# valauri/Littoral-Naval-Warfare-MARL

Hardware: AMD Instinct MI355X
Metric: env-steps/sec (whole node), 65536 parallel 4v4 envs on 100x100 grid (higher is better)
Workload: dtype f64+i32; 1 GPU; 65536 parallel 4v4 envs over 1 GPU(s) (65536 on rank 0), 100x100 Baltic grid, reference spawns, 40-step episodes with auto-reset, U[0,1)^4 f32 actions; global_envs=65536, envs_per_gpu=65536, agents=4v4, grid=100, spawns=reference, kernel_variant=default, los_mode=0, move_mode=0, parallelism=env-shard x1

## Files before the change

littoral-naval-warfare-marl_amd/csrc/lnw_device.h:

```cpp
#pragma once
#include <hip/hip_runtime.h>
#include <stdint.h>

namespace lnw {

constexpr int WAVE = 64;
constexpr int R_MV = 4;
constexpr int MV_W = 2 * R_MV + 1;
constexpr int MV_WORDS = 3;
constexpr int R_LOS = 40;
constexpr int LOS_W = 2 * R_LOS + 1;
constexpr int LOS_ROW_WORDS = 6;
constexpr int LOS_CELL_WORDS = LOS_W * LOS_ROW_WORDS;
constexpr int OPEN_CAP = 16;

enum { K_PYINT = 0, K_PYFLOAT = 1, K_F32 = 2, K_F64 = 3 };
enum { T_SMALL = 0, T_LARGE = 1, T_LS = 2, T_MEDIUM = 3 };

constexpr double PY_PI = 3.141592653589793;
constexpr double RAD2DEG = 180.0 / PY_PI;
constexpr double DEG2RAD = PY_PI / 180.0;

struct KParams {
  int discrete, landing_ops, aggressive, side_blue, trained_red;
  int move_thr, ew_thr, lz_x, lz_y;
  int episode_steps, auto_reset, los_mode, move_mode;
  int E, nb, nr, A, G, T, W16;
  int rng_mode;
  int act_dtype;
  int rew_f64;
  long long env_base;
  unsigned long long seed;
  double red_aggression;
  double hit64[2][9];
  float hit32[2][9];
  double d5[2][2];
  double den[2];
  double det_q[2];
  int box_lo[2], box_hi[2];
  int group_march;
  int xcd_remap;
  int wc[2];
  int epw;
  int store_wt;
  int atan_odd;
  int no_obs;
  long long obs_stride[2];
  int dbg_skip;
  int qdirect;
};

struct KState {
  uint32_t *pos;
  int32_t *radar;
  uint8_t *miss;
  uint8_t *mkind;
  uint8_t *alive;
  uint8_t *type;
  int32_t *steps;
  double *dist_lz;
  uint16_t *tl_cnt;
  uint16_t *tl;
  double *duct;
  int32_t *envi;
  unsigned long long *rng;
  uint32_t *err;
  double *bear_val;
  uint8_t *bear_ship;
  const double *atan_deg;
  const uint8_t *grid;
  const float *gridf;
  const float *winf;
  float *dummy;
  unsigned long long *prof;
  lnw_analytics ana;
  unsigned long long *ctr;
  const uint32_t *mask2;
  const uint32_t *mvtab;
  const uint32_t *lostab;
  const double *tape;
  const long long *tape_off;
  const int32_t *sp_types;
  const int32_t *sp_pos;
  const int32_t *sp_randls;
  const int32_t *sp_pos_env;
  int nmax;
};

__host__ __device__ inline uint32_t pack_pos(int x, int y) {
  return (uint32_t)(x & 0xffff) | ((uint32_t)(y & 0xffff) << 16);
}
__device__ inline int pos_x(uint32_t p) { return (int)(p & 0x7fff); }
__device__ inline int pos_y(uint32_t p) { return (int)((p >> 16) & 0x7fff); }

__device__ inline int kind_promote(int a, int b) {
  if (a == K_F64 || b == K_F64) return K_F64;
  if (a == K_F32 || b == K_F32) return K_F32;
  if (a == K_PYFLOAT || b == K_PYFLOAT) return K_PYFLOAT;
  return K_PYINT;
}

__device__ inline void philox10(uint32_t c[4], uint32_t k0, uint32_t k1) {
#pragma unroll
  for (int r = 0; r < 10; r++) {
    uint32_t hi0 = __umulhi(0xD2511F53u, c[0]), lo0 = 0xD2511F53u * c[0];
    uint32_t hi1 = __umulhi(0xCD9E8D57u, c[2]), lo1 = 0xCD9E8D57u * c[2];
    uint32_t n0 = hi1 ^ c[1] ^ k0, n2 = hi0 ^ c[3] ^ k1;
    c[0] = n0; c[1] = lo1; c[2] = n2; c[3] = lo0;
    k0 += 0x9E3779B9u;
    k1 += 0xBB67AE85u;
  }
}

__device__ inline void philox_u4(unsigned long long seed, unsigned long long ctr, float (&u)[4]) {
  uint32_t o[4] = {(uint32_t)ctr, (uint32_t)(ctr >> 32), 0x243F6A88u, 0x85A308D3u};
  philox10(o, (uint32_t)seed, (uint32_t)(seed >> 32));
#pragma unroll
  for (int k = 0; k < 4; k++) u[k] = (float)(o[k] >> 8) * 5.9604644775390625e-08f;
}

__device__ inline double u53(uint32_t a, uint32_t b) {
  return ((double)(a >> 5) * 67108864.0 + (double)(b >> 6)) / 9007199254740992.0;
}

__host__ __device__ inline unsigned long long tan_bits(double x) { return __builtin_bit_cast(unsigned long long, x); }
__host__ __device__ inline double tan_from_bits(unsigned long long b) { return __builtin_bit_cast(double, b); }
__host__ __device__ inline double tan_kernel_fd(double x, double y, int iy) {
  const double T0 = 3.33333333333334091986e-01, T1 = 1.33333333333201242699e-01,
               T2 = 5.39682539762260521377e-02, T3 = 2.18694882948595424599e-02,
               T4 = 8.86323982359930005737e-03, T5 = 3.59207910759131235356e-03,
               T6 = 1.45620945432529025516e-03, T7 = 5.88041240820264096874e-04,
               T8 = 2.46463134818469906812e-04, T9 = 7.81794442939557092300e-05,
               T10 = 7.14072491382608190305e-05, T11 = -1.85586374855275456654e-05,
               T12 = 2.59073051863633712884e-05;
  const double pio4 = 7.85398163397448278999e-01, pio4lo = 3.06161699786838301793e-17;
  const int hx = (int)(tan_bits(x) >> 32), ix = hx & 0x7fffffff;
  if (ix < 0x3e300000) {
    if (iy == 1) return x;
    return -1.0 / x;
  }
  const bool big = ix >= 0x3FE59428;
  if (big) {
    if (hx < 0) { x = -x; y = -y; }
    const double z = pio4 - x, w = pio4lo - y;
    x = z + w;
    y = 0.0;
  }
  double z = x * x, w = z * z;
  double r = T1 + w * (T3 + w * (T5 + w * (T7 + w * (T9 + w * T11))));
  double v = z * (T2 + w * (T4 + w * (T6 + w * (T8 + w * (T10 + w * T12)))));
  double s = z * x;
  r = y + z * (s * (r + v) + y);
  r += T0 * s;
  w = x + r;
  if (big) {
    v = (double)iy;
    return (double)(1 - ((hx >> 30) & 2)) * (v - 2.0 * (x - (w * w / (w + v) - r)));
  }
  if (iy == 1) return w;
  const double zz = tan_from_bits(tan_bits(w) & 0xffffffff00000000ull);
  v = r - (zz - x);
  const double a = -1.0 / w;
  const double t = tan_from_bits(tan_bits(a) & 0xffffffff00000000ull);
  s = 1.0 + t * zz;
  return t + a * (s + t * v);
}
__host__ __device__ inline double tan_fd(double x) {
  const int ix = (int)(tan_bits(x) >> 32) & 0x7fffffff;
// ... 395 lines not shown
```

littoral-naval-warfare-marl_amd/csrc/lnw_group.inc:

```

#ifdef LNW_GROUP_PROF
#define GPROF_MARK(t) unsigned long long t = __builtin_amdgcn_s_memrealtime()
#define GPROF_SET(t) (t) = __builtin_amdgcn_s_memrealtime()
#define GPROF_ADD(X, k, t)                                                   \
  do {                                                                       \
    const unsigned long long _n = __builtin_amdgcn_s_memrealtime();          \
    (X).gp[k] += _n - (t);                                                   \
    (t) = _n;                                                                \
  } while (0)
#define GPROF_FLUSH(X)                                                       \
  do {                                                                       \
    if ((X).S.prof && (threadIdx.x & (WAVE - 1)) == 0)                        \
      for (int _k = 0; _k < 8; _k++)                                         \
        atomicAdd(&(X).S.prof[(size_t)blockIdx.x * PROF_SLOTS + 16 + _k], (X).gp[_k]); \
  } while (0)
#else
#define GPROF_MARK(t) (void)0
#define GPROF_SET(t) (void)0
#define GPROF_ADD(X, k, t) (void)0
#define GPROF_FLUSH(X) (void)0
#endif

constexpr int GL = 16;
constexpr int GEPW = 32;
// ... 256 lines not shown
  g.pos = side ? gs[1].pos : gs[0].pos;
  g.shared = side ? gs[1].shared : gs[0].shared;
  const int jj = sub;
  const uint32_t posj = g.pos;
  const int gsh = (int)(threadIdx.x & (WAVE - 1)) & ~(GL - 1);
  GPROF_MARK(tq);
  const int ml = me - own0;
  const uint32_t vm = (movedm >> own0) & ((2u << ml) - 1u) & 0xffffu;
  auto sel = [&](uint32_t b) { return ((b & 0xffffu) & ~vm) | ((b >> 16) & vm); };
  const bool myradar = COLW(c.radar_cur, me) == 1;
  const bool nowalk = P.dbg_skip & 8192;
  const uint32_t dcol = nowalk ? 0u : (sel(g.c) | (myradar ? sel(g.r) : 0u));
  const uint32_t ecol = nowalk ? 0u : sel(g.w);
  GPROF_ADD(X, 4, tq);
  const int INF = 0x7fffffff;
  const int ij = dcol ? __builtin_ctz(dcol) : -1;
  int gj = ij >= 0 ? ij * nopp + jj : INF;
  if (g.shared) {
    int grow = -1, gcol = 0;
    for (uint32_t rows = group_or(dcol); rows; rows &= rows - 1) {
      const int i = __builtin_ctz(rows);
      const uint32_t m = group_ballot((dcol >> i) & 1u, gsh) & g.mates;
      if (grow < 0 && m) { grow = i; gcol = __builtin_ctz(m); }
    }
    gj = grow >= 0 ? grow * nopp + gcol : INF;
  }
  const bool rep = ij >= 0 && ij * nopp + jj == gj;
  const uint32_t low = (1u << jj) - 1u;
  const unsigned long long base = X.rng.ctr;
  auto slope_at = [&](int i, uint32_t pj, int r) {
    const uint32_t pi = COLW(c.pos_cur, own0 + i);
    const double a0 = bearing_tab(P, atab, half, pos_x(pj) - pos_x(pi), pos_y(pj) - pos_y(pi));
    const double gd = (P.dbg_skip & 262144) ? (double)(r & 7) * 0.25 - 1.0
                                            : X.rng.gauss_at(base + (unsigned long long)r);
    const double bearing = a0 + gd < 0 ? a0 + gd + 360.0 : a0 + gd;
    return (P.dbg_skip & 524288) ? bearing * 0.01 : tan_fd(bearing * DEG2RAD);
  };

  int nbear = 0, obs_n = 0, orank = 0, n = 0;
  uint32_t colb = 0;
  uint64_t it0 = 0, it1 = 0;
  int ni = 0;
  for (uint32_t rows = group_or(ecol | (rep ? 1u << ij : 0u)); rows; rows &= rows - 1) {
    const int i = __builtin_ctz(rows);
    const bool bb = ((ecol >> i) & 1u) && i * nopp + jj < gj;
    const uint32_t brow = group_ballot(bb, gsh);
    if (bb) {
      n++;
      colb |= 1u << i;
    }
    {
      const int cnt = __builtin_popcount(brow), t = (sub - nbear) & (GL - 1);
      if (t < cnt) {
        uint32_t mm = brow;
        int pos = 0, kk = t, cc = __builtin_popcount(mm & 0xffu);
        if (kk >= cc) { kk -= cc; mm >>= 8; pos += 8; }
        cc = __builtin_popcount(mm & 0xfu);
        if (kk >= cc) { kk -= cc; mm >>= 4; pos += 4; }
        cc = __builtin_popcount(mm & 0x3u);
        if (kk >= cc) { kk -= cc; mm >>= 2; pos += 2; }
        if (kk >= (int)(mm & 1u)) pos += 1;
        const uint64_t item = (uint64_t)(i | pos << 4 | ((nbear + t) & 0xff) << 8);
        if (ni < 4) it0 |= item << (16 * ni);
        else if (ni < 8) it1 |= item << (16 * (ni - 4));
        else ms[(i * nopp + pos) * GEPW] = slope_at(i, COLW(c.pos_cur, opp0 + pos), nbear + t);
        ni++;
      }
    }
    nbear += __builtin_popcount(brow);
    const bool rr = rep && ij == i;
    const uint32_t rrow = group_ballot(rr, gsh);
    if (rr) orank = obs_n + __builtin_popcount(rrow & low);
    obs_n += __builtin_popcount(rrow);
  }
  if (X.rng.mode == 1) {
    const long long avail = X.rng.tape_hi - X.rng.tape_lo - (long long)base;
    if (nbear > avail) X.rng.err |= 4u;
    X.rng.ctr += (unsigned long long)(nbear < avail ? nbear : (avail > 0 ? avail : 0));
  } else {
    X.rng.ctr += (unsigned long long)nbear;
  }
  GPROF_ADD(X, 5, tq);
  const uint32_t fixm = group_ballot(n >= 2, gsh);
  if (S.ctr && n >= 2) X.pooled += (unsigned)n;
  if (fixm && !(P.dbg_skip & 16384)) {
    auto item = [&](int q) { return (uint32_t)((q < 4 ? it0 >> (16 * q) : it1 >> (16 * (q - 4))) & 0xffffu); };
    for (int q = 0; q < ni; q += 2) {
      const uint32_t u1 = item(q), u2 = q + 1 < ni ? item(q + 1) : 0u;
      const bool f1 = (fixm >> ((u1 >> 4) & 15u)) & 1u, f2 = q + 1 < ni && ((fixm >> ((u2 >> 4) & 15u)) & 1u);
      if (!f1 && !f2) continue;
      const uint32_t v1 = f1 ? u1 : u2, v2 = f1 && f2 ? u2 : v1;
      const double m1 = slope_at((int)(v1 & 15u), COLW(c.pos_cur, opp0 + ((v1 >> 4) & 15u)), (int)(v1 >> 8));
      const double m2 = slope_at((int)(v2 & 15u), COLW(c.pos_cur, opp0 + ((v2 >> 4) & 15u)), (int)(v2 >> 8));
      ms[((v1 & 15u) * nopp + ((v1 >> 4) & 15u)) * GEPW] = m1;
      if (f1 && f2) ms[((v2 & 15u) * nopp + ((v2 >> 4) & 15u)) * GEPW] = m2;
    }
    wave_lds_sync();
  }
  const int fb = colb ? __builtin_ctz(colb) * nopp + jj : INF;
  int nt = 0, fxi = 0, fyi = 0;
  uint32_t err = 0;
  if (n >= 2 && !(P.dbg_skip & 16384)) {
    auto slope = [&](int i, double &x1, double &y1) {
      const uint32_t pi = COLW(c.pos_cur, own0 + i);
      x1 = pos_x(pi);
      y1 = pos_y(pi);
      return ms[(i * nopp + jj) * GEPW];
    };
    const int m = n - 1;
    FixAcc16 f;
    bool zero = false;
    double mprev = 0.0, xprev = 0.0, yprev = 0.0;
    uint32_t bits = colb;
    int k = 0;
    auto take = [&](double mt, double x1, double y1) {
      if (k > 0 && !zero) {
        if (mprev - mt == 0.0) {
          zero = true;
        } else {
          double x3, y3;
          fix_pair(mprev, mt, xprev, yprev, x1, y1, x3, y3);
          f.add(k - 1, m, x3, y3);
        }
      }
      k++;
      mprev = mt;
      xprev = x1;
      yprev = y1;
    };
    while (bits && !zero) {
      const int i1 = __builtin_ctz(bits);
      bits &= bits - 1;
      const bool two = bits != 0;
      const int i2 = two ? __builtin_ctz(bits) : i1;
      if (two) bits &= bits - 1;
      double x1, y1, x2, y2;
      const double m1 = slope(i1, x1, y1), m2 = slope(i2, x2, y2);
      take(m1, x1, y1);
      if (two) take(m2, x2, y2);
    }
    {
      double mx = 0.0, my = 0.0;
      if (zero) {
        err |= LNW_ERRF_ZERODIV;
      } else {
        f.mean(m, mx, my);
        if (!isfinite(mx) || !isfinite(my)) {
          err |= LNW_ERRF_NAN_ROUND;
        } else {
          const double rx = rint(mx), ry = rint(my);
          if (S.ana.ew_log) {
            const int ax = (int)fmin(fmax(rx, -32768.0), 32767.0), ay = (int)fmin(fmax(ry, -32768.0), 32767.0);
            ana_record(S.ana.ew_log, S.ana.ew_count, S.ana.ew_cap, (uint32_t)(P.env_base + env),
                       (uint32_t)X.step | (uint32_t)side << 16, COLW(c.pos_cur, me),
                       (uint32_t)(uint16_t)ax | (uint32_t)(uint16_t)ay << 16);
          }
          if (rx >= 0.0 && rx < (double)P.G && ry >= 0.0 && ry < (double)P.G) {
            fxi = (int)rx;
            fyi = (int)ry;
            for (int q = opp0; q < opp1; q++) {
              if (!COLB(c.alive0, q)) continue;
              const uint32_t pq = COLW(c.pos_cur, q);
              const int ddx = pos_x(pq) - fxi, ddy = pos_y(pq) - fyi;
              nt += ddx * ddx + ddy * ddy < 4 ? 1 : 0;
            }
          }
        }
      }
    }
  }
  GPROF_ADD(X, 6, tq);
  int off = obs_n, tot = obs_n;
#pragma unroll
  for (int q = 0; q < GL; q++) {
    const int fbg = __shfl(fb, gsh + q), ntg = __shfl(nt, gsh + q);
    tot += ntg;
    off += fbg < fb ? ntg : 0;
  }
  uint16_t *tl = S.tl + (size_t)me * P.T * E + env;
  const bool tls = !(P.dbg_skip & 1048576);
  if (rep && tls) tl[(size_t)orank * E] = (uint16_t)(pos_x(posj) | (pos_y(posj) << 8));
  if (nt > 0 && tls) {
    for (int q = opp0; q < opp1; q++) {
      if (!COLB(c.alive0, q)) continue;
      const uint32_t pq = COLW(c.pos_cur, q);
      const int ddx = pos_x(pq) - fxi, ddy = pos_y(pq) - fyi;
      if (ddx * ddx + ddy * ddy < 4) {
        tl[(size_t)off * E] = (uint16_t)(fxi | (fyi << 8));
        off++;
      }
    }
  }
  COLW(c.tcnt, me) = (uint32_t)tot;
  X.rng.err |= group_or(err);
  GPROF_ADD(X, 7, tq);
}

__device__ __forceinline__ float row_tail(const KParams &P, const Cols &c, const double *duct_col,
                                          int el, int k, int tk, uint32_t p, int own0, int ns,
                                          int kl, int t) {
  const double G = (double)P.G;
  if (t < 4) {
    if (t == 0) return (float)((double)pos_x(p) / G);
    if (t == 1) return (float)((double)pos_y(p) / G);
    if (t == 2) return (float)c.radar_cur[k * PAD + el];
    return (float)c.miss_cur[k * PADB + el] * (tk == T_SMALL ? 0.25f : 0.125f);
  }
  t -= 4;
  if (t < 4 * (ns - 1)) {
    const int s = t >> 2, comp = t & 3;
    const int il = s < kl ? s : s + 1, i = own0 + il;
    if (!c.alive0[i * PADB + el]) return 0.0f;
    const bool nw = il < kl;
    const uint32_t q = nw ? c.pos_cur[i * PAD + el] : c.pos_old[i * PAD + el];
    if (comp == 0) return (float)((double)pos_x(q) / G);
    if (comp == 1) return (float)((double)pos_y(q) / G);
    if (comp == 2) return (float)(nw ? c.radar_cur[i * PAD + el] : c.radar_old[i * PAD + el]);
    const int m = nw ? c.miss_cur[i * PADB + el] : c.miss_old[i * PADB + el];
    return (float)m * (c.type[i * PADB + el] == T_SMALL ? 0.25f : 0.125f);
  }
  t -= 4 * (ns - 1);
  if (t == 0) return (float)c.tcnt[k * PAD + el];
  if (t == 1) return tk == T_LS ? 1.0f : 0.0f;
  if (t == 2) return (float)(duct_col[el] / 2.0);
  return 0.0f;
}

__device__ __forceinline__ void group_rows(const KParams &P, const KState &S, const Cols &c,
                                           const double *duct_col, int el, long long env, int sub,
                                           float *obs_b, float *obs_r) {
  for (int sd = 0; sd < 2; sd++) {
    float *out = sd ? obs_r : obs_b;
    if (!out) continue;
    const int own0 = sd ? P.nb : 0, ns = sd ? P.nr : P.nb;
    const int D = side_D(P, sd), D4 = D / 4;
    f32x4 *base = (f32x4 *)(out + (size_t)env * ns * D);
// ... 109 lines not shown
  }
  if (tid < GEPW) {
    const double d = tid < nenv ? S.duct[env0 + tid] : 1.0;
    duct_col[tid] = d;
    r2col[tid] = max_range2(P, d);
  }
  __syncthreads();
  if (tid == 0) prof_stamp(S, 4);

  const int dt = P.act_dtype;
  bool pend = false;
  if (dt == LNW_ACT_F32)
    pend = group_move_phase<LNW_ACT_F32>(P, S, c, actions, row_kind, c.mask, env0, nenv, A, wid);
  else if (dt == LNW_ACT_F64)
    pend = group_move_phase<LNW_ACT_F64>(P, S, c, actions, row_kind, c.mask, env0, nenv, A, wid);
  else
    pend = group_move_phase<LNW_ACT_I32>(P, S, c, actions, row_kind, c.mask, env0, nenv, A, wid);
  if (__syncthreads_or(pend)) {
    if (wid == 0) move_astar_pass(P, S, c, nenv, A);
    __syncthreads();
  }

  if (tid == 0) prof_stamp(S, 1);
  if (valid) {
    Ctx X{P, S, c, slot, env, duct_col, make_rng(P, S, env), c.mask, E, r2col[slot], 0};
    X.leader = sub == 0;
    X.gsub = sub;
    X.gsh = (int)(threadIdx.x & (WAVE - 1)) & ~(GL - 1);
    GSide gs[2];
    uint32_t movedm;
    GPROF_MARK(tp);
    group_pair_tables(X, sub, gs, movedm);
    GPROF_ADD(X, 3, tp);
    Neut N{{0, 0}, {0u, 0u}};
    int ev[8];
#pragma unroll
    for (int q = 0; q < 8; q++) ev[q] = S.envi[q * E + env];
    X.step = ev[2];
    int hits[2] = {0, 0};
    int bsx = 0, bsy = 0, rsx = 0, rsy = 0;
    int nbp = 0, nrp = 0;
    GPROF_MARK(t0);
    for (int a = 0; a < A; a++) {
      const int lane = slot;
      const bool al = COLB(c.alive0, a) != 0;
      const int side = a >= nb;
      bool engage = false, moved = false;
      int destroyed = 0;
      if (al) {
        const uint32_t p0 = COLW(c.pos_cur, a);
        if (!side) {
          if (P.side_blue) { bsx += pos_x(p0); bsy += pos_y(p0); nbp++; }
        } else {
          rsx += pos_x(p0); rsy += pos_y(p0); nrp++;
        }
        const size_t row = ((size_t)env * A + a) * 4;
        const double a0 = COLW(c.act0, a);
        double a1 = COLW(c.act1, a);
        const int kind = COLB(c.akind, a);
        if (side && !P.trained_red) {
          if (X.rng.uniform() < P.red_aggression) {
            double v = X.rng.uniform();
            if (dt == LNW_ACT_F32) { float f = (float)v; ((float *)actions)[row + 1] = f; a1 = f; }
            else if (dt == LNW_ACT_F64) {
              if (kind == K_F32) v = (double)(float)v;
              ((double *)actions)[row + 1] = v; a1 = v;
            } else { ((int32_t *)actions)[row + 1] = 0; a1 = 0.0; }
          }
        }
        const double engagement = P.discrete ? rint(a1) : a1;
        const int keng = P.discrete ? K_PYINT : kind;
        const int mk = COLB(c.mkind, a);
        double thr_v;
        if (kind_promote(keng, mk) == K_F32)
          thr_v = (double)rintf((float)engagement * (float)COLB(c.miss_cur, a));
        else
          thr_v = rint(engagement * (double)COLB(c.miss_cur, a));
        if (!isfinite(thr_v)) { X.rng.err |= LNW_ERRF_NAN_ROUND; thr_v = 0.0; }
        engage = thr_v > 0.0;
        const int tn = (int)COLW(c.tcnt, a);
        if (engage && tn > 0 && !(P.dbg_skip & 65536)) {
          const uint16_t *tl = S.tl + (size_t)a * P.T * E + env;
          const int gsh = (int)(threadIdx.x & (WAVE - 1)) & ~(GL - 1);
          const bool par = !S.ana.heatmap && !S.ana.coldmap && !S.ana.launch && !S.ana.eng_log &&
                           !(P.dbg_skip & 32768);
          for (int q0 = 0; q0 < tn; q0 += GL) {
            const int q = q0 + sub;
            const int mine = q >= tn ? 0 : (tls && q < GTL) ? (int)tls[(a * GTL + q) * GEPW + slot]
                                                           : (int)tl[(size_t)q * E];
            const int nq = tn - q0 < GL ? tn - q0 : GL;
            if (par) {
              destroyed += fire_group_chunk(X, a, mine, nq, engagement, keng, N);
              continue;
            }
            for (int u = 0; u < nq; u++) {
              const uint16_t tg = (uint16_t)__shfl(mine, gsh + u);
              if (fire_dev<true>(X, a, tg & 0xff, tg >> 8, engagement, keng, N)) destroyed++;
            }
          }
        }
        if (side) ev[6] += destroyed; else ev[5] += destroyed;
        if (!isfinite(a0)) { X.rng.err |= LNW_ERRF_NAN_ROUND; COLW(c.radar_cur, a) = 0; }
        else {
          const double rr = rint(a0);
          COLW(c.radar_cur, a) = (int)fmin(fmax(rr, -2147483648.0), 2147483647.0);
        }
        const uint32_t pn = COLW(c.pos_new, a);
        moved = (pn & 0x80000000u) != 0;
        if (moved) COLW(c.pos_cur, a) = pn & 0x7fffffffu;
        GPROF_ADD(X, 0, t0);
        if (!(P.dbg_skip & 128)) get_obs_group(X, a, sub, gs, movedm, atab, half, ms);
        GPROF_SET(t0);
      }
      double r = 0.0;
      if (al && !(P.dbg_skip & 256))
        r = reward_core(P, S, c, slot, E, env, a, moved, engage, destroyed, dlz ? dlz + slot : nullptr, GEPW);
      GPROF_ADD(X, 1, t0);
      COLW(c.reward, a) = r;
      if (al) {
        if (!side) {
          if (P.side_blue ? destroyed > 0 : engage) COLB(c.eng, a) = 1;
        } else {
          if (!P.trained_red ? engage : destroyed > 1) COLB(c.eng, a) = 1;
        }
        if (side) hits[1] += destroyed; else hits[0] += destroyed;
      }
    }
    env_tail(P, S, c, slot, env, nb, A, N, ev, hits, nbp, nrp, bsx, bsy, rsx, rsy, X.rng, rew_b,
             rew_r, done_out, cog_out);
    if (S.ctr && X.pooled) atomicAdd(&S.ctr[3], (unsigned long long)X.pooled);
    GPROF_ADD(X, 2, t0);
    GPROF_FLUSH(X);
  }
  if (valid && !(P.dbg_skip & 1) && !P.no_obs) group_rows(P, S, c, duct_col, slot, env, sub, obs_b, obs_r);
}
```

littoral-naval-warfare-marl_amd/csrc/lnw_kernels.hip:

```cpp
#include <hip/hip_runtime.h>

#include <algorithm>
#include <cmath>
#include <cstdio>
#include <cstdlib>
#include <cstring>
#include <string>
#include <vector>

#include "lnw.h"
#include "lnw_device.h"

using namespace lnw;

typedef float f32x4 __attribute__((ext_vector_type(4)));
typedef int i32x4_t __attribute__((ext_vector_type(4)));

__device__ __forceinline__ void st_obs4(f32x4 *base, uint32_t i4, f32x4 v, bool wt) {
  if (wt) {
    const uint64_t bp = (uint64_t)(uintptr_t)base;
    const uint64_t ub = (uint64_t)(uint32_t)__builtin_amdgcn_readfirstlane((int)(uint32_t)bp) |
                        (uint64_t)(uint32_t)__builtin_amdgcn_readfirstlane((int)(uint32_t)(bp >> 32)) << 32;
    const __amdgpu_buffer_rsrc_t rs =
        __builtin_amdgcn_make_buffer_rsrc((void *)(uintptr_t)ub, 0, 0x7fffffff, 0x00020000);
// ... 141 lines not shown
  c.qstage1 = (float *)(base + L.qstage1);
  c.qlut = (float *)(base + L.qlut);
  c.qbig = (float *)(base + L.qbig);
  return c;
}

#define COLW(arr, a) ((arr)[(a) * PAD + lane])
#define COLB(arr, a) ((arr)[(a) * PADB + lane])

constexpr int PROF_SLOTS = 32;
__device__ inline unsigned long long prof_now(const KState &S) {
  return S.prof ? __builtin_amdgcn_s_memrealtime() : 0ull;
}
__device__ inline unsigned long long prof_acc(const KState &S, int slot, unsigned long long t0) {
  if (!S.prof) return 0ull;
  const unsigned long long t = __builtin_amdgcn_s_memrealtime();
  const unsigned long long m = __ballot(1);
  if ((int)(threadIdx.x & 63) == __ffsll((long long)m) - 1)
    atomicAdd(&S.prof[(size_t)blockIdx.x * PROF_SLOTS + slot], t - t0);
  return t;
}

struct Ctx {
  const KParams &P;
  const KState &S;
  Cols &c;
  int lane, env;
  const double *duct_col;
  Rng rng;
  const uint32_t *mask;
  long long E;
  int r2max;
  int step;
  uint64_t lpre[2];
  bool pre;
  uint32_t ptr_[2] = {0u, 0u}, ptc[2] = {0u, 0u}, ptw[2] = {0u, 0u};
  bool leader = true;
  int gsub = 0, gsh = 0;
  unsigned pooled = 0;
#ifdef LNW_GROUP_PROF
  unsigned long long gp[8] = {0, 0, 0, 0, 0, 0, 0, 0};
#endif
  __device__ double duct() const { return duct_col[lane]; }
};

__device__ inline void ana_record(uint32_t *log, uint32_t *count, long long cap, uint32_t w0,
                                  uint32_t w1, uint32_t w2, uint32_t w3) {
  const uint32_t i = atomicAdd(count, 1u);
  if ((long long)i < cap) {
    uint4 *r = (uint4 *)log + i;
    *r = make_uint4(w0, w1, w2, w3);
  }
}
__device__ inline void ana_map(uint32_t *map, uint32_t p) {
  const int x = pos_x(p), y = pos_y(p);
  if (map && x < 100 && y < 100) atomicAdd(&map[x * 100 + y], 1u);
}

__device__ inline int max_range2(const KParams &P, double duct) {
  int m = 16;
  for (int ti = 0; ti < 3; ti++)
    for (int tj = 0; tj < 3; tj++) {
      int r = radar_r(P, duct, ti, tj), e = ew_r(P, duct, ti, tj);
      m = max(m, max(r * r, e * e));
    }
  return m;
}

__device__ inline int floordiv7(int v) { int q = v / 7; if ((v % 7 != 0) && (v < 0)) q--; return q; }
__device__ inline int pymod7(int v) { int m = v % 7; if (m < 0) m += 7; return m; }

__device__ inline bool check_path_h(const KParams &P, const KState &S, int type, int sx, int sy,
                                    int tx, int ty, uint32_t *open, int ost) {
  if (tx < 0 || tx > 99 || ty < 0 || ty > 99) return false;
  int ox = tx - sx, oy = ty - sy;
  if (P.move_mode == 0 && ox >= -R_MV && ox <= R_MV && oy >= -R_MV && oy <= R_MV) {
    int cls = mv_cls(type);
    int bit = (ox + R_MV) * MV_W + (oy + R_MV);
    uint32_t w = S.mvtab[((size_t)cls * P.G * P.G + (size_t)sx * P.G + sy) * MV_WORDS + (bit >> 5)];
    return (w >> (bit & 31)) & 1u;
  }
  MaskBlocked mb{S.mask2, P.W16};
  bool sb = mb(sx, sy);
  if (S.ctr) atomicAdd(&S.ctr[2], 1ull);
  return check_path_dev(mb, sb, P.G, type, sx, sy, tx, ty, open, ost);
}

__device__ inline bool can_move_to_h(const KParams &P, const KState &S, int x, int y) {
  if (0 <= x && x < 100 && 0 <= y && y < 100) return !(cell_bits(S.mask2, P.W16, x, y) & 1u);
  return false;
}

__device__ inline uint32_t los_march_c(const KState &S, const uint32_t *mask, int W16, int x1,
                                       int y1, int x2, int y2) {
  if (!S.ctr) return los_march<true>(mask, W16, x1, y1, x2, y2);
  int n = 0;
  const uint32_t r = los_march<true>(mask, W16, x1, y1, x2, y2, &n);
  atomicAdd(&S.ctr[0], 1ull);
  atomicAdd(&S.ctr[1], (unsigned long long)n);
  return r;
}

__device__ inline uint32_t los_q(const KParams &P, const KState &S, const uint32_t *mask, int x1,
                                 int y1, int x2, int y2) {
  int dx = x2 - x1, dy = y2 - y1;
  if (P.los_mode != 1 && dx >= -R_LOS && dx <= R_LOS && dy >= -R_LOS && dy <= R_LOS) {
    int col = (dy + R_LOS) * 2;
    uint32_t w = S.lostab[((size_t)x1 * P.G + y1) * LOS_CELL_WORDS + (dx + R_LOS) * LOS_ROW_WORDS +
                          (col >> 5)];
    return (w >> (col & 31)) & 3u;
  }
  return los_march_c(S, mask, P.W16, x1, y1, x2, y2);
}

struct ObsAcc {
  int obs_n, norder;
};

__device__ inline void pair_after_los(Ctx &X, int i, int jj, int xi, int yi, int xj, int yj,
                                      bool rad_ok, bool close, bool ew_cand, uint32_t los,
                                      ObsAcc &acc);

__device__ inline void pair_detect(Ctx &X, int myradar, int i, int jj, int xi, int yi, int ti,
                                   int xj, int yj, int tj, int radj, int d2, ObsAcc &acc) {
  const KParams &P = X.P;
  const KState &S = X.S;
  Cols &c = X.c;
  const int lane = X.lane;
  int rr = radar_r(P, X.duct(), ti, tj), re = ew_r(P, X.duct(), ti, tj);
  bool rad_ok = myradar == 1 && d2 < rr * rr;
  bool close = d2 < 16;
  bool ew_cand = d2 < re * re && radj == 1;
  if (!(rad_ok || close || ew_cand)) return;
  pair_after_los(X, i, jj, xi, yi, xj, yj, rad_ok, close, ew_cand,
                 los_q(P, S, X.mask, xi, yi, xj, yj), acc);
}

__device__ inline bool pair_observe(Ctx &X, int xj, int yj, bool rad_ok, bool close, bool ew_cand,
                                    uint32_t los, ObsAcc &acc) {
  Cols &c = X.c;
  const int lane = X.lane;
  if (!(los & 1u)) return false;
  uint32_t pk = pack_pos(xj, yj);
  bool seen = false;
  for (int q = 0; q < acc.obs_n; q++) seen |= COLW(c.observed, q) == pk;
  if ((rad_ok || close) && !seen) {
    COLW(c.observed, acc.obs_n) = pk;
    acc.obs_n++;
    seen = true;
  }
  return ew_cand && (los & 2u) && !seen;
}

__device__ inline double bearing_deg(const KParams &P, const KState &S, int dx, int dy) {
  const bool tab = !(P.dbg_skip & 4096) && S.atan_deg && dx >= -R_LOS && dx <= R_LOS &&
                   dy >= -R_LOS && dy <= R_LOS;
  return tab ? S.atan_deg[(dy + R_LOS) * LOS_W + (dx + R_LOS)] : atan2((double)dy, (double)dx) * RAD2DEG;
}

struct BearPre {
  double v;
  bool tab;
};
__device__ inline BearPre bearing_pre(const KParams &P, const KState &S, int dx, int dy) {
  const bool tab = !(P.dbg_skip & 4096) && S.atan_deg && dx >= -R_LOS && dx <= R_LOS &&
                   dy >= -R_LOS && dy <= R_LOS;
  const double *p = tab ? S.atan_deg + (dy + R_LOS) * LOS_W + (dx + R_LOS) : (const double *)S.dummy;
  return {*p, tab};
}
__device__ inline double bearing_use(const BearPre &b, int dx, int dy) {
  return b.tab ? b.v : atan2((double)dy, (double)dx) * RAD2DEG;
}

__device__ inline double ew_bearing(const KParams &P, const KState &S, int xi, int yi, int xj, int yj,
                                    double distortion) {
  double bearing = bearing_deg(P, S, xj - xi, yj - yi);
  if (bearing + distortion < 0)
    bearing = bearing + distortion + 360.0;
  else
    bearing = bearing + distortion;
  return bearing;
}

__device__ inline void pair_after_los(Ctx &X, int i, int jj, int xi, int yi, int xj, int yj,
                                      bool rad_ok, bool close, bool ew_cand, uint32_t los,
                                      ObsAcc &acc) {
  const KState &S = X.S;
  Cols &c = X.c;
  const int lane = X.lane;
  if (pair_observe(X, xj, yj, rad_ok, close, ew_cand, los, acc)) {
    const double bearing = ew_bearing(X.P, S, xi, yi, xj, yj, X.rng.gauss());
    int k = COLB(c.bcnt, jj);
    if (k == 0) { COLB(c.border, acc.norder) = (uint8_t)jj; acc.norder++; }
    size_t slot = (size_t)(jj * S.nmax + k) * X.E + X.env;
    S.bear_val[slot] = bearing;
    S.bear_ship[slot] = (uint8_t)i;
    COLB(c.bcnt, jj) = (uint8_t)(k + 1);
  }
}

__device__ inline void pair_after_los_m(Ctx &X, int i, int jj, int opp0, int nopp, int xi, int yi,
                                        int xj, int yj, bool rad_ok, bool close, bool ew_cand,
                                        uint32_t los, ObsAcc &acc, uint64_t &obsm) {
  const KState &S = X.S;
  Cols &c = X.c;
  const int lane = X.lane;
  if (!(los & 1u)) return;
  bool seen = (obsm >> jj) & 1u;
  if ((rad_ok || close) && !seen) {
    const uint32_t pk = pack_pos(xj, yj);
    COLW(c.observed, acc.obs_n) = pk;
    acc.obs_n++;
    for (int k = 0; k < nopp; k++)
      if (COLW(c.pos_cur, opp0 + k) == pk) obsm |= 1ull << k;
    seen = true;
  }
  if (ew_cand && (los & 2u) && !seen) {
    const double bearing = ew_bearing(X.P, S, xi, yi, xj, yj, X.rng.gauss());
    int k = COLB(c.bcnt, jj);
    if (k == 0) { COLB(c.border, acc.norder) = (uint8_t)jj; acc.norder++; }
    size_t slot = (size_t)(jj * S.nmax + k) * X.E + X.env;
    S.bear_val[slot] = bearing;
    S.bear_ship[slot] = (uint8_t)i;
    COLB(c.bcnt, jj) = (uint8_t)(k + 1);
  }
}

struct FixAcc {
  double sumx = 0, sumy = 0, resx = 0, resy = 0;
  double r0x = 0, r1x = 0, r2x = 0, r3x = 0, r4x = 0, r5x = 0, r6x = 0, r7x = 0;
  double r0y = 0, r1y = 0, r2y = 0, r3y = 0, r4y = 0, r5y = 0, r6y = 0, r7y = 0;
  bool tail_started = false;
  __device__ void put(int r, bool acc, double x3, double y3) {
#define LNW_PUT(i)                                              \
  r##i##x = r == i ? (acc ? r##i##x + x3 : x3) : r##i##x;      \
  r##i##y = r == i ? (acc ? r##i##y + y3 : y3) : r##i##y;
    LNW_PUT(0) LNW_PUT(1) LNW_PUT(2) LNW_PUT(3) LNW_PUT(4) LNW_PUT(5) LNW_PUT(6) LNW_PUT(7)
#undef LNW_PUT
  }
  __device__ void add(int k, int m, double x3, double y3) {
    const int mblk = m - (m % 8);
    if (m < 8) {
      sumx += x3;
      sumy += y3;
    } else if (k < mblk) {
      put(k & 7, k >= 8, x3, y3);
    } else {
      if (!tail_started) { tree(); tail_started = true; }
      resx += x3;
      resy += y3;
    }
  }
  __device__ void tree() {
    resx = ((r0x + r1x) + (r2x + r3x)) + ((r4x + r5x) + (r6x + r7x));
    resy = ((r0y + r1y) + (r2y + r3y)) + ((r4y + r5y) + (r6y + r7y));
  }
  __device__ void mean(int m, double &mx, double &my) {
    if (m < 8) { mx = sumx / (double)m; my = sumy / (double)m; return; }
    if (!tail_started) tree();
    mx = resx / (double)m;
    my = resy / (double)m;
  }
};

__device__ inline void fix_pair(double m1, double m2, double x1, double y1, double x2, double y2,
                                double &x3, double &y3) {
  x3 = (m1 * x1 - m2 * x2 + y2 - y1) / (m1 - m2);
  y3 = m1 * (x3 - x1) + y1;
}

__device__ inline bool fix_mean_loop(Ctx &X, int jj, int n, double &mx, double &my) {
  const KState &S = X.S;
  Cols &c = X.c;
  const int lane = X.lane;
  auto slot = [&](int k) { return (size_t)(jj * S.nmax + k) * X.E + X.env; };
  const int m = n - 1;
  FixAcc f;
  for (int k = 0; k < m; k++) {
    uint8_t s1 = S.bear_ship[slot(k)], s2 = S.bear_ship[slot(k + 1)];
    double b1 = S.bear_val[slot(k)], b2 = S.bear_val[slot(k + 1)];
    uint32_t p1 = COLW(c.pos_cur, s1), p2 = COLW(c.pos_cur, s2);
    double m1 = tan_fd(b1 * DEG2RAD);
    double m2 = tan_fd(b2 * DEG2RAD);
    if (m1 - m2 == 0.0) return false;
    double x3, y3;
    fix_pair(m1, m2, pos_x(p1), pos_y(p1), pos_x(p2), pos_y(p2), x3, y3);
    f.add(k, m, x3, y3);
  }
  f.mean(m, mx, my);
  return true;
}

template <int BMAX>
__device__ inline bool fix_mean_batched(Ctx &X, int jj, int n, double &mx, double &my) {
  const KState &S = X.S;
  Cols &c = X.c;
  const int lane = X.lane;
  auto slot = [&](int k) { return (size_t)(jj * S.nmax + k) * X.E + X.env; };
  double bv[BMAX];
  int bs[BMAX];
#pragma unroll
  for (int k = 0; k < BMAX; k++) {
    bv[k] = 0.0;
    bs[k] = 0;
    if (k < n) { bv[k] = S.bear_val[slot(k)]; bs[k] = S.bear_ship[slot(k)]; }
  }
  double tv[BMAX], px[BMAX], py[BMAX];
#pragma unroll
  for (int k = 0; k < BMAX; k++) {
    tv[k] = 0.0;
    px[k] = py[k] = 0.0;
    if (k < n) {
      tv[k] = tan_fd(bv[k] * DEG2RAD);
      const uint32_t p = COLW(c.pos_cur, bs[k]);
      px[k] = pos_x(p);
      py[k] = pos_y(p);
    }
  }
  const int m = n - 1;
  FixAcc f;
  bool zero = false;
#pragma unroll
  for (int k = 0; k < BMAX - 1; k++) {
    if (k < m && !zero) {
      if (tv[k] - tv[k + 1] == 0.0) {
        zero = true;
      } else {
        double x3, y3;
        fix_pair(tv[k], tv[k + 1], px[k], py[k], px[k + 1], py[k + 1], x3, y3);
        f.add(k, m, x3, y3);
      }
    }
  }
  if (zero) return false;
  f.mean(m, mx, my);
  return true;
}

template <int BMAX, bool EXACT>
__device__ inline void finish_obs(Ctx &X, int me, int opp0, int opp1, const ObsAcc &acc) {
  const KParams &P = X.P;
  const KState &S = X.S;
  Cols &c = X.c;
  const int lane = X.lane;
  const long long E = X.E;
  const int env = X.env;
  const int obs_n = acc.obs_n, norder = acc.norder;
  const int T = P.T;
  uint16_t *tl = S.tl + (size_t)me * T * E + env;
  int tn = 0;
  for (int q = 0; q < obs_n; q++) {
    uint32_t pk = COLW(c.observed, q);
    tl[(size_t)tn * E] = (uint16_t)(pos_x(pk) | (pos_y(pk) << 8));
    tn++;
  }
  for (int o = 0; o < norder; o++) {
    int jj = COLB(c.border, o);
    int n = COLB(c.bcnt, jj);
    if (n < 2) continue;
    double mx, my;
    bool ok;
    if constexpr (EXACT) ok = fix_mean_batched<BMAX>(X, jj, n, mx, my);
    else ok = n <= BMAX ? fix_mean_batched<BMAX>(X, jj, n, mx, my) : fix_mean_loop(X, jj, n, mx, my);
    if (!ok) { X.rng.err |= LNW_ERRF_ZERODIV; continue; }
    if (!isfinite(mx) || !isfinite(my)) { X.rng.err |= LNW_ERRF_NAN_ROUND; continue; }
    double rx = rint(mx), ry = rint(my);
    if (S.ana.ew_log) {
      const int fx = (int)fmin(fmax(rx, -32768.0), 32767.0), fy = (int)fmin(fmax(ry, -32768.0), 32767.0);
      ana_record(S.ana.ew_log, S.ana.ew_count, S.ana.ew_cap, (uint32_t)(P.env_base + env),
                 (uint32_t)X.step | (uint32_t)(me >= P.nb) << 16, COLW(c.pos_cur, me),
                 (uint32_t)(uint16_t)fx | (uint32_t)(uint16_t)fy << 16);
    }
    if (!(rx >= 0.0 && rx < (double)P.G && ry >= 0.0 && ry < (double)P.G)) continue;
    int fxi = (int)rx, fyi = (int)ry;
    for (int j = opp0; j < opp1; j++) {
      if (!COLB(c.alive0, j)) continue;
      uint32_t pj = COLW(c.pos_cur, j);
      int ddx = pos_x(pj) - fxi, ddy = pos_y(pj) - fyi;
      if (ddx * ddx + ddy * ddy < 4) {
        tl[(size_t)tn * E] = (uint16_t)(fxi | (fyi << 8));
        tn++;
      }
    }
  }
  COLW(c.tcnt, me) = (uint32_t)tn;
}


template <int N, class T>
__device__ __forceinline__ T rsel(const T (&a)[N], int k) {
  T v = a[0];
#pragma unroll
  for (int q = 1; q < N; q++) v = k == q ? a[q] : v;
  return v;
}

__device__ __forceinline__ void march_pairs_ref(Ctx &X, int me) {
  const KParams &P = X.P;
  const Cols &c = X.c;
  const int lane = X.lane;
  const int side = me >= P.nb;
  const int own0 = side ? P.nb : 0, own1 = side ? P.A : P.nb;
  const int opp0 = side ? 0 : P.nb, opp1 = side ? P.nb : P.A;
  uint32_t acc = 0;
  for (int i = own0; i < own1; i++) {
    if (!COLB(c.alive0, i)) continue;
    const uint32_t pi = COLW(c.pos_cur, i);
    for (int j = opp0; j < opp1; j++) {
      if (!COLB(c.alive0, j)) continue;
      const uint32_t pj = COLW(c.pos_cur, j);
      int n = 0;
      acc += los_march<false>(X.mask, P.W16, pos_x(pi), pos_y(pi), pos_x(pj), pos_y(pj), &n);
      if (X.S.ctr) {
        atomicAdd(&X.S.ctr[0], 1ull);
        atomicAdd(&X.S.ctr[1], (unsigned long long)n);
      }
    }
  }
  if (acc == 0xffffffffu) X.S.dummy[lane] = 0.0f;
}

__device__ __forceinline__ void get_obs_dev(Ctx &X, int me) {
  const KParams &P = X.P;
  const KState &S = X.S;
  Cols &c = X.c;
  const int lane = X.lane;
  const int nb = P.nb, A = P.A;
  const int side = me >= nb;
  const int own0 = side ? nb : 0, own1 = side ? A : nb;
  const int opp0 = side ? 0 : nb, opp1 = side ? nb : A;
  const int nopp = opp1 - opp0, npair = (own1 - own0) * nopp;
  const int myradar = COLW(c.radar_cur, me);
  ObsAcc acc{0, 0};
  uint64_t obsm = 0;
  for (int q = 0; q < nopp; q++) COLB(c.bcnt, q) = 0;
  const double duct = X.duct();
  int rr_t[2][3], re_t[2][3];
#pragma unroll
  for (int mi = 0; mi < 2; mi++)
#pragma unroll
    for (int tj = 0; tj < 3; tj++) {
      const int ti = mi ? T_LARGE : T_SMALL;
      rr_t[mi][tj] = radar_r(P, duct, ti, tj);
      re_t[mi][tj] = ew_r(P, duct, ti, tj);
    }
  const unsigned long long tw = prof_now(S);
#pragma unroll 1
  for (int b0 = 0; b0 < npair; b0 += 16) {
    uint32_t radm = 0, closem = 0, ewm = 0, tabm = 0, marchm = 0;
    uint32_t wi[16];
    int ic = own0 + b0 / nopp, jc = opp0 + b0 % nopp;
    bool al_i = COLB(c.alive0, ic);
    uint32_t pi_c = COLW(c.pos_cur, ic);
    int mi_c = mast_cls(COLB(c.type, ic));
#pragma unroll
    for (int u = 0; u < 16; u++) {
      wi[u] = 0;
      const int b = b0 + u;
      const int j = jc;
      const bool ali = al_i;
      const uint32_t pi = pi_c;
      const int mi = mi_c;
      if (++jc == opp1) {
        jc = opp0;
        if (++ic < own1) {
          al_i = COLB(c.alive0, ic);
          pi_c = COLW(c.pos_cur, ic);
          mi_c = mast_cls(COLB(c.type, ic));
        }
      }
      if (b >= npair) continue;
      if (!ali || !COLB(c.alive0, j)) continue;
      const uint32_t pj = COLW(c.pos_cur, j);
      const int dx = pos_x(pj) - pos_x(pi), dy = pos_y(pj) - pos_y(pi);
      const int d2 = dx * dx + dy * dy;
      if (d2 >= X.r2max) continue;
      const int tj = rng_cls(COLB(c.type, j));
      const int rr0 = tj == 0 ? rr_t[0][0] : (tj == 1 ? rr_t[0][1] : rr_t[0][2]);
      const int rr1 = tj == 0 ? rr_t[1][0] : (tj == 1 ? rr_t[1][1] : rr_t[1][2]);
      const int re0 = tj == 0 ? re_t[0][0] : (tj == 1 ? re_t[0][1] : re_t[0][2]);
      const int re1 = tj == 0 ? re_t[1][0] : (tj == 1 ? re_t[1][1] : re_t[1][2]);
      const int rr = mi ? rr1 : rr0, re = mi ? re1 : re0;
      const bool rad_ok = myradar == 1 && d2 < rr * rr, close = d2 < 16;
      const bool ew_cand = d2 < re * re && COLW(c.radar_cur, j) == 1;
      if (!(rad_ok || close || ew_cand)) continue;
      radm |= (rad_ok ? 1u : 0u) << u;
      closem |= (close ? 1u : 0u) << u;
      ewm |= (ew_cand ? 1u : 0u) << u;
      if (P.los_mode != 1 && dx >= -R_LOS && dx <= R_LOS && dy >= -R_LOS && dy <= R_LOS) {
        tabm |= 1u << u;
        wi[u] = ((uint32_t)(pos_x(pi) * P.G + pos_y(pi)) * LOS_CELL_WORDS + (dx + R_LOS) * LOS_ROW_WORDS) *
                    32u + (dy + R_LOS) * 2;
      } else {
        marchm |= 1u << u;
      }
    }
    uint32_t losb = 0;
#pragma unroll
// ... 16 lines not shown
    }
  }
  const unsigned long long tf = prof_acc(S, 20, tw);
  finish_obs<16, false>(X, me, opp0, opp1, acc);
  prof_acc(S, 22, tf);
}


template <int NOWN, int NOPP, bool CW>
__device__ inline void finish_obs_t(Ctx &X, int me, int own0, int opp0, int obs_n,
                                    uint32_t firstbit, uint32_t bearm,
                                    const uint32_t (&pp)[NOPP], uint32_t oal = 0) {
  static_assert(NOWN < 9, "np.mean pairwise summation starts at 8 terms");
  const KParams &P = X.P;
  const KState &S = X.S;
  Cols &c = X.c;
  const int lane = X.lane;
  const long long E = X.E;
  const int env = X.env;
  const unsigned long long base = X.rng.ctr;
  const int nbear = __builtin_popcount(bearm);
  if (X.rng.mode == 1) {
    const long long avail = X.rng.tape_hi - X.rng.tape_lo - (long long)base;
    if (nbear > avail) X.rng.err |= 4u;
    X.rng.ctr += (unsigned long long)(nbear < avail ? nbear : (avail > 0 ? avail : 0));
  } else {
    X.rng.ctr += (unsigned long long)nbear;
  }
  uint16_t *tl = S.tl + (size_t)me * P.T * E + env;
  unsigned long long tq = prof_now(S);
  int tn = 0;
  if constexpr (CW) {
    for (uint32_t fb = firstbit; fb; fb &= fb - 1) {
      const uint32_t pk = COLW(c.pos_cur, opp0 + __builtin_ctz(fb) % NOPP);
      tl[(size_t)tn * E] = (uint16_t)(pos_x(pk) | (pos_y(pk) << 8));
      tn++;
    }
  } else {
    for (int q = 0; q < obs_n; q++) {
      uint32_t pk = COLW(c.observed, q);
      tl[(size_t)tn * E] = (uint16_t)(pos_x(pk) | (pos_y(pk) << 8));
      tn++;
    }
  }
  tq = prof_acc(S, 21, tq);
  if (!CW && bearm == 0) { COLW(c.tcnt, me) = (uint32_t)tn; return; }
  uint32_t colj = 0;
#pragma unroll
  for (int i = 0; i < NOWN; i++) colj |= 1u << (i * NOPP);
  uint32_t need = 0;
#pragma unroll
  for (int j = 0; j < NOPP; j++) {
    const uint32_t bj = bearm & (colj << j);
    if (__builtin_popcount(bj) < 2) continue;
#pragma unroll
    for (int i = 0; i < NOWN; i++) need |= ((bj >> (i * NOPP + j)) & 1u) << (j * NOWN + i);
  }
  if (S.prof) {
    const int cnt = __builtin_popcount(need);
    int s = 0, mx = 0;
    for (int b = 4; b >= 0; b--) {
      s += __popcll(__ballot((cnt >> b) & 1)) << b;
      if (__ballot(cnt >= (mx | (1 << b)))) mx |= 1 << b;
    }
    const unsigned long long m = __ballot(1);
    if ((int)(threadIdx.x & 63) == __ffsll((long long)m) - 1) {
      atomicAdd(&S.prof[(size_t)blockIdx.x * PROF_SLOTS + 24], (unsigned long long)s);
      atomicAdd(&S.prof[(size_t)blockIdx.x * PROF_SLOTS + 25], (unsigned long long)mx);
      atomicAdd(&S.prof[(size_t)blockIdx.x * PROF_SLOTS + 26], (unsigned long long)__popcll(m));
    }
  }
  static_assert(NOPP <= 4, "fix cells packed 16 bits per opponent");
  uint64_t fixw = 0;
  uint32_t fok = 0;
  int curj = -1, cnt = 0;
  bool zero = false;
  double sumx = 0.0, sumy = 0.0, mprev = 0.0, xprev = 0.0, yprev = 0.0;
  auto flush = [&]() {
    if (curj < 0) return;
    if (zero) { X.rng.err |= LNW_ERRF_ZERODIV; return; }
    const double mx = sumx / (double)(cnt - 1), my = sumy / (double)(cnt - 1);
    if (!isfinite(mx) || !isfinite(my)) { X.rng.err |= LNW_ERRF_NAN_ROUND; return; }
    const double rx = rint(mx), ry = rint(my);
    if (S.ana.ew_log) {
      const int fx = (int)fmin(fmax(rx, -32768.0), 32767.0), fy = (int)fmin(fmax(ry, -32768.0), 32767.0);
      ana_record(S.ana.ew_log, S.ana.ew_count, S.ana.ew_cap, (uint32_t)(P.env_base + env),
                 (uint32_t)X.step | (uint32_t)(me >= P.nb) << 16, COLW(c.pos_cur, me),
                 (uint32_t)(uint16_t)fx | (uint32_t)(uint16_t)fy << 16);
    }
    if (!(rx >= 0.0 && rx < (double)P.G && ry >= 0.0 && ry < (double)P.G)) return;
    fixw |= (uint64_t)((uint32_t)(int)rx | (uint32_t)(int)ry << 8) << (16 * curj);
    fok |= 1u << curj;
  };
  if constexpr (CW) {
  auto setup = [&](int t, int &dx, int &dy, int &j, double &x1, double &y1, int &k) {
    j = t / NOWN;
    const int i = t - j * NOWN, b = i * NOPP + j;
    const uint32_t pi = COLW(c.pos_cur, own0 + i), pj = COLW(c.pos_cur, opp0 + j);
    dx = pos_x(pj) - pos_x(pi);
    dy = pos_y(pj) - pos_y(pi);
    x1 = pos_x(pi);
    y1 = pos_y(pi);
    k = __builtin_popcount(bearm & ((1u << b) - 1u));
  };
  auto accum = [&](int j, double m, double x1, double y1) {
    if (j != curj) {
      flush();
      curj = j; cnt = 0; zero = false; sumx = sumy = 0.0;
    }
    if (cnt > 0 && !zero) {
      if (mprev - m == 0.0) {
        zero = true;
      } else {
        double x3, y3;
        fix_pair(mprev, m, xprev, yprev, x1, y1, x3, y3);
        sumx += x3;
        sumy += y3;
      }
    }
    cnt++;
    mprev = m; xprev = x1; yprev = y1;
  };
  const unsigned long long act = __ballot(1);
  const int ncnt = __builtin_popcount(need);
  int wmax = 0;
#pragma unroll
  for (int b = 4; b >= 0; b--)
    if (__ballot(ncnt >= (wmax | (1 << b)))) wmax |= 1 << b;
  if (NOWN * NOPP > 2 && wmax > 2 && !(P.dbg_skip & 131072)) {
    const int nact = __popcll(act);
    const int rank = (int)__builtin_amdgcn_mbcnt_hi((uint32_t)(act >> 32),
                                                    __builtin_amdgcn_mbcnt_lo((uint32_t)act, 0u));
    int excl = 0, total = 0;
#pragma unroll
    for (int b = 0; b < 5; b++) {
      const unsigned long long bb = __ballot((ncnt >> b) & 1);
      excl += (int)__builtin_amdgcn_mbcnt_hi((uint32_t)(bb >> 32),
                                             __builtin_amdgcn_mbcnt_lo((uint32_t)bb, 0u)) << b;
      total += __popcll(bb) << b;
    }
    if (S.ctr && rank == 0) atomicAdd(&S.ctr[3], (unsigned long long)total);
    uint8_t *lor = (uint8_t *)c.observed;
    uint16_t *exr = (uint16_t *)(lor + WAVE);
    uint32_t *fixt = (uint32_t *)(lor + 3 * WAVE);
    lor[rank] = (uint8_t)lane;
    exr[rank] = (uint16_t)excl;
    asm volatile("s_waitcnt lgkmcnt(0)" ::: "memory");
    const int prevl = rank > 0 ? (int)lor[rank - 1] : lane;
    const int lastl = 63 - __builtin_clzll(act);
    const bool tape = X.rng.mode == 1;
    constexpr uint32_t SEGM = (1u << NOWN) - 1u;
    auto locate = [&](int g, int &s, int &i, int &j, uint32_t &nsj, unsigned long long &drw,
                      uint32_t &pi, uint32_t &pj) {
      int lo = 0;
#pragma unroll
      for (int st = 32; st; st >>= 1)
        if (lo + st < nact && (int)exr[lo + st] <= g) lo += st;
      s = lor[lo];
      const int kk = g - (int)exr[lo];
      uint32_t ns = (uint32_t)__shfl((int)need, s);
      const uint32_t bs = (uint32_t)__shfl((int)bearm, s);
      drw = __shfl(base, s);
      uint32_t w = ns;
      for (int q = 0; q < kk; q++) w &= w - 1;
      const int t = __builtin_ctz(w);
      j = t / NOWN;
      i = t - j * NOWN;
      const int b = i * NOPP + j;
      drw += (unsigned long long)__builtin_popcount(bs & ((1u << b) - 1u));
      nsj = (ns >> (j * NOWN)) & SEGM;
      pi = c.pos_cur[(own0 + i) * PAD + s];
      pj = c.pos_cur[(opp0 + j) * PAD + s];
    };
    auto draw = [&](int s, unsigned long long d) -> double {
      const int es = env - lane + s;
      if (tape) {
        if (!S.tape_off) return 0.0;
        const long long p = S.tape_off[es] + (long long)d;
        return p < S.tape_off[es + 1] ? S.tape[p] : 0.0;
      }
      const unsigned long long gid = (unsigned long long)(P.env_base + es);
      return X.rng.gauss_philox(d, (uint32_t)gid, (uint32_t)(gid >> 32));
    };
    auto finish = [&](int s, int j, int n, double sx, double sy, bool z, int stp) {
      uint32_t w = 0;
      if (z) {
        w = 1u << 17;
      } else {
        const double mx = sx / (double)(n - 1), my = sy / (double)(n - 1);
        if (!isfinite(mx) || !isfinite(my)) {
          w = 1u << 18;
        } else {
          const double rx = rint(mx), ry = rint(my);
          if (S.ana.ew_log) {
            const int fx = (int)fmin(fmax(rx, -32768.0), 32767.0), fy = (int)fmin(fmax(ry, -32768.0), 32767.0);
            ana_record(S.ana.ew_log, S.ana.ew_count, S.ana.ew_cap, (uint32_t)(P.env_base + env - lane + s),
                       (uint32_t)stp | (uint32_t)(me >= P.nb) << 16, c.pos_cur[me * PAD + s],
                       (uint32_t)(uint16_t)fx | (uint32_t)(uint16_t)fy << 16);
          }
          if (rx >= 0.0 && rx < (double)P.G && ry >= 0.0 && ry < (double)P.G)
            w = (uint32_t)(int)rx | (uint32_t)(int)ry << 8 | 1u << 16;
        }
      }
      fixt[j * WAVE + s] = w;
    };
    double cm = 0.0, csx = 0.0, csy = 0.0;
    uint32_t cp = 0;
    int cz = 0;
    for (int r0 = 0; r0 < total; r0 += 2 * nact) {
      const int gA = r0 + 2 * rank, gB = gA + 1;
      int sA, iA, jA, sB, iB, jB;
      uint32_t nA, nB, piA, pjA, piB, pjB;
      unsigned long long dA, dB;
      locate(min(gA, total - 1), sA, iA, jA, nA, dA, piA, pjA);
      locate(min(gB, total - 1), sB, iB, jB, nB, dB, piB, pjB);
      const int dx1 = pos_x(pjA) - pos_x(piA), dy1 = pos_y(pjA) - pos_y(piA);
      const int dx2 = pos_x(pjB) - pos_x(piB), dy2 = pos_y(pjB) - pos_y(piB);
      const BearPre b1 = bearing_pre(P, S, dx1, dy1), b2 = bearing_pre(P, S, dx2, dy2);
      double a1 = b1.v, a2 = b2.v;
      if (!(b1.tab && b2.tab)) {
        a1 = bearing_use(b1, dx1, dy1);
        a2 = bearing_use(b2, dx2, dy2);
      }
      const double gg1 = draw(sA, dA), gg2 = draw(sB, dB);
      const double br1 = a1 + gg1 < 0 ? a1 + gg1 + 360.0 : a1 + gg1;
      const double br2 = a2 + gg2 < 0 ? a2 + gg2 + 360.0 : a2 + gg2;
      const double mA = tan_fd(br1 * DEG2RAD), mB = tan_fd(br2 * DEG2RAD);
      const bool fA = !(nA & ((1u << iA) - 1u)), fB = !(nB & ((1u << iB) - 1u));
      const bool lA = !(nA >> (iA + 1)), lB = !(nB >> (iB + 1));
      const double tm = __shfl(mB, prevl);
      const uint32_t tp = (uint32_t)__shfl((int)piB, prevl);
      const double pm = rank > 0 ? tm : cm;
      const uint32_t pp = rank > 0 ? tp : cp;
      double xA = 0.0, yA = 0.0, xB = 0.0, yB = 0.0;
      const bool zA = !fA && pm - mA == 0.0, zB = !fB && mA - mB == 0.0;
      if (!fA && !zA)
        fix_pair(pm, mA, pos_x(pp), pos_y(pp), pos_x(piA), pos_y(piA), xA, yA);
      if (!fB && !zB)
        fix_pair(mA, mB, pos_x(piA), pos_y(piA), pos_x(piB), pos_y(piB), xB, yB);
      double sxA = 0.0, syA = 0.0, sxB = 0.0, syB = 0.0;
      bool ZA = false, ZB = false;
#pragma unroll
      for (int pass = 0; pass < (NOWN - 1) / 2 + 1; pass++) {
        const double qx = __shfl(sxB, prevl), qy = __shfl(syB, prevl);
        const int qz = __shfl((int)ZB, prevl);
        const double inx = rank > 0 ? qx : csx, iny = rank > 0 ? qy : csy;
        const bool inz = (rank > 0 ? qz : cz) != 0;
        sxA = fA ? 0.0 : inx + xA;
        syA = fA ? 0.0 : iny + yA;
        ZA = !fA && (inz || zA);
        sxB = fB ? 0.0 : sxA + xB;
        syB = fB ? 0.0 : syA + yB;
        ZB = !fB && (ZA || zB);
      }
      int stA = 0, stB = 0;
      if (S.ana.ew_log) {
        stA = __shfl(X.step, sA);
        stB = __shfl(X.step, sB);
      }
      if (gA < total && lA) finish(sA, jA, __builtin_popcount(nA), sxA, syA, ZA, stA);
      if (gB < total && lB) finish(sB, jB, __builtin_popcount(nB), sxB, syB, ZB, stB);
      cm = __shfl(mB, lastl);
      cp = (uint32_t)__shfl((int)piB, lastl);
      csx = __shfl(sxB, lastl);
      csy = __shfl(syB, lastl);
      cz = __shfl((int)ZB, lastl);
    }
    asm volatile("s_waitcnt lgkmcnt(0)" ::: "memory");
#pragma unroll
    for (int j = 0; j < NOPP; j++) {
      if (__builtin_popcount((need >> (j * NOWN)) & SEGM) < 2) continue;
      const uint32_t w = fixt[j * WAVE + lane];
      if (w & (1u << 17)) X.rng.err |= LNW_ERRF_ZERODIV;
      else if (w & (1u << 18)) X.rng.err |= LNW_ERRF_NAN_ROUND;
      else if (w & (1u << 16)) {
        fixw |= (uint64_t)(w & 0xffffu) << (16 * j);
        fok |= 1u << j;
      }
    }
  } else
  while (need) {
    const int t1 = __builtin_ctz(need);
    need &= need - 1;
    const bool two = need != 0;
    const int t2 = two ? __builtin_ctz(need) : t1;
    if (two) need &= need - 1;
    int dx1, dy1, j1, k1, dx2, dy2, j2, k2;
    double x1, y1, x2, y2;
    setup(t1, dx1, dy1, j1, x1, y1, k1);
    setup(t2, dx2, dy2, j2, x2, y2, k2);
    const BearPre b1 = bearing_pre(P, S, dx1, dy1), b2 = bearing_pre(P, S, dx2, dy2);
    double a1 = b1.v, a2 = b2.v;
    if (!(b1.tab && b2.tab)) {
      a1 = bearing_use(b1, dx1, dy1);
      a2 = bearing_use(b2, dx2, dy2);
    }
    const double g1 = X.rng.gauss_at(base + (unsigned long long)k1);
    const double g2 = X.rng.gauss_at(base + (unsigned long long)k2);
    const double br1 = a1 + g1 < 0 ? a1 + g1 + 360.0 : a1 + g1;
    const double br2 = a2 + g2 < 0 ? a2 + g2 + 360.0 : a2 + g2;
    const double m1 = tan_fd(br1 * DEG2RAD), m2 = tan_fd(br2 * DEG2RAD);
    accum(j1, m1, x1, y1);
    if (two) accum(j2, m2, x2, y2);
  }
  } else {
  while (need) {
    const int t = __builtin_ctz(need);
    need &= need - 1;
    const int j = t / NOWN, i = t - j * NOWN, b = i * NOPP + j;
    const uint32_t pi = COLW(c.pos_cur, own0 + i), pj = COLW(c.pos_cur, opp0 + j);
    const int dx = pos_x(pj) - pos_x(pi), dy = pos_y(pj) - pos_y(pi);
    const double a0 = bearing_deg(P, S, dx, dy);
    if (j != curj) {
      flush();
      curj = j; cnt = 0; zero = false; sumx = sumy = 0.0;
    }
    const int k = __builtin_popcount(bearm & ((1u << b) - 1u));
    const double g = X.rng.gauss_at(base + (unsigned long long)k);
    const double bearing = a0 + g < 0 ? a0 + g + 360.0 : a0 + g;
    const double m = tan_fd(bearing * DEG2RAD);
    const double x1 = pos_x(pi), y1 = pos_y(pi);
    if (cnt > 0 && !zero) {
      if (mprev - m == 0.0) {
        zero = true;
      } else {
        double x3, y3;
        fix_pair(mprev, m, xprev, yprev, x1, y1, x3, y3);
        sumx += x3;
        sumy += y3;
      }
    }
    cnt++;
    mprev = m; xprev = x1; yprev = y1;
  }
  }
  flush();
  tq = prof_acc(S, 22, tq);
  uint32_t rem = bearm, done = 0;
  while (rem) {
// ... 366 lines not shown
template <bool GRP = false>
__device__ inline int check_target_dev(Ctx &X, int side, int tx, int ty) {
  const KParams &P = X.P;
  Cols &c = X.c;
  const int lane = X.lane;
  int opp0 = side ? 0 : P.nb, opp1 = side ? P.nb : P.A;
  if constexpr (GRP) {
    const int j = opp0 + X.gsub;
    bool hit = false;
    if (j < opp1 && COLB(c.alive0, j)) {
      const uint32_t pj = COLW(c.pos_cur, j);
      const int dx = pos_x(pj) - tx, dy = pos_y(pj) - ty;
      hit = dx * dx + dy * dy <= 12;
    }
    const uint32_t m = (uint32_t)(__ballot(hit) >> X.gsh) & 0xffffu;
    return m ? opp0 + __builtin_ctz(m) : -1;
  }
  for (int j = opp0; j < opp1; j++) {
    if (!COLB(c.alive0, j)) continue;
    uint32_t pj = COLW(c.pos_cur, j);
    int dx = pos_x(pj) - tx, dy = pos_y(pj) - ty;
    if (dx * dx + dy * dy <= 12) return j;
  }
  return -1;
}

struct Neut {
  int cnt[2];
  uint32_t mask[2];
};

template <bool GRP = false>
__device__ inline bool fire_dev(Ctx &X, int a, int tx, int ty, double salvo, int ksalvo, Neut &N) {
  const KParams &P = X.P;
  Cols &c = X.c;
  const int lane = X.lane;
  const int side = a >= P.nb;
  int t = check_target_dev<GRP>(X, side, tx, ty);
  if (t < 0) return false;
  uint32_t pt = COLW(c.pos_cur, t), pa = COLW(c.pos_cur, a);
  int dx = pos_x(pt) - pos_x(pa), dy = pos_y(pt) - pos_y(pa);
  bool hit = false, missile = false;
  int n = 0;
  if (dx * dx + dy * dy < 4) {
    hit = true;
  } else {
    int miss = COLB(c.miss_cur, a);
    if (miss == 0) return false;
    int mk = COLB(c.mkind, a);
    double u1, u2;
    X.rng.uniform2(u1, u2);
    bool detected = !(u1 < (COLW(c.radar_cur, t) == 1 ? P.det_q[0] : P.det_q[1]));
    int hp = detected ? 0 : 1;
    double num;
    int kn;
    if (!P.discrete) {
      int kp = kind_promote(mk, ksalvo);
      if (kp == K_F32) {
        num = (double)rintf((float)miss * (float)salvo);
        kn = K_F32;
      } else {
        num = rint((double)miss * salvo);
        kn = K_F64;
      }
    } else {
      num = COLB(c.type, a) == T_SMALL ? salvo : salvo * 2.0;
      kn = K_PYINT;
    }
    if (num > (double)miss) { num = (double)miss; kn = mk; }
    n = (int)num;
    COLB(c.miss_cur, a) = (uint8_t)(miss - n);
    COLB(c.mkind, a) = (uint8_t)kind_promote(mk, kn);
    if (n < 0 || n > 8) { X.rng.err |= LNW_ERRF_MISSILES; n = n < 0 ? 0 : 8; }
    if (kn == K_F32)
      hit = (float)u2 < hit_sel(P.hit32, hp, n);
    else
      hit = u2 < hit_sel(P.hit64, hp, n);
    missile = true;
  }
  if (hit && X.leader) {
    const KState &S = X.S;
    if (missile) {
      if (side == (P.side_blue ? 0 : 1)) {
        ana_map(S.ana.heatmap, pa);
        ana_map(S.ana.coldmap, pt);
      }
      if (S.ana.launch) ana_map(S.ana.launch + side * 10000, pa);
    }
    if (S.ana.eng_log)
      ana_record(S.ana.eng_log, S.ana.eng_count, S.ana.eng_cap, (uint32_t)(P.env_base + X.env),
                 (uint32_t)X.step | (uint32_t)side << 16 | (uint32_t)n << 24, pa, pt);
  }
  if (hit) {
    int ts = t >= P.nb;
    N.cnt[ts]++;
    N.mask[ts] |= 1u << (t - (ts ? P.nb : 0));
  }
  return hit;
}

__device__ inline int fire_draws(Ctx &X, int a, double salvo, int ksalvo) {
  const KParams &P = X.P;
  Cols &c = X.c;
  const int lane = X.lane;
  const int side = a >= P.nb;
  const int tn = (int)COLW(c.tcnt, a);
  int miss = COLB(c.miss_cur, a), mk = COLB(c.mkind, a), nd = 0;
  const uint16_t *tl = X.S.tl + (size_t)a * P.T * X.E + X.env;
  const uint32_t pa = COLW(c.pos_cur, a);
  for (int q = 0; q < tn; q++) {
    const uint16_t tg = tl[(size_t)q * X.E];
    const int t = check_target_dev<false>(X, side, tg & 0xff, tg >> 8);
    if (t < 0) continue;
    const uint32_t pt = COLW(c.pos_cur, t);
    const int dx = pos_x(pt) - pos_x(pa), dy = pos_y(pt) - pos_y(pa);
    if (dx * dx + dy * dy < 4 || miss == 0) continue;
    double num;
    int kn;
    if (!P.discrete) {
      if (kind_promote(mk, ksalvo) == K_F32) {
        num = (double)rintf((float)miss * (float)salvo);
        kn = K_F32;
      } else {
        num = rint((double)miss * salvo);
        kn = K_F64;
      }
    } else {
      num = COLB(c.type, a) == T_SMALL ? salvo : salvo * 2.0;
      kn = K_PYINT;
    }
    if (num > (double)miss) { num = (double)miss; kn = mk; }
    miss = (miss - (int)num) & 0xff;
    mk = kind_promote(mk, kn);
    nd += 2;
  }
  return nd;
}

__device__ __forceinline__ double reward_core(const KParams &P, const KState &S, Cols &c, int lane,
                                              long long E, int env, int a, bool moved, bool engage,
                                              int n_hit, const double *dlz = nullptr, int dlz_stride = 0) {
  size_t ai = (size_t)a * E + env;
  int steps = COLW(c.steps, a) + 1;
  COLW(c.steps, a) = steps;
  int tl_n = (int)COLW(c.tcnt, a);
  double r = 0.0;
  if (tl_n > 0) r += (double)(tl_n * 3);
  if (moved) r += 1.0;
  else r = fmax(r - 0.5, 0.0);
  if (tl_n > 0 && !engage) r = r / 2.0;
  else if (tl_n > 0 && engage && n_hit == 0) r += 0.5;
  r += (double)(n_hit * 10);
  int t = COLB(c.type, a);
  uint32_t p = COLW(c.pos_cur, a);
  int x = pos_x(p), y = pos_y(p);
  bool red = a >= P.nb;
  if (red && t != T_LS && !P.aggressive) {
    if (steps > 14) {
      if (x < 19 || x > 55 || y < 40 || y > 70) r = fmax(r - 2.0, 0.0);
      else r += 1.0;
    }
  }
  if (red && P.aggressive && t != T_LS) {
    int dx = x - 15, dy = y - 60;
    double nom = fmax(sqrt((double)(dx * dx + dy * dy)), 1.0);
    double d = (1.0 / (nom / (mast_cls(t) ? P.den[1] : P.den[0]))) * 1.0;
    r += d;
  }
  if (t == T_LS) {
    int dx = x - P.lz_x, dy = y - P.lz_y;
    double dl = sqrt((double)(dx * dx + dy * dy));
    if (dl > 0) {
      double cur = (P.dbg_skip & 2097152) ? 1e9 : (dlz ? dlz[a * dlz_stride] : S.dist_lz[ai]);
      if (dl < cur) { r += 1.0; S.dist_lz[ai] = dl; }
      else r -= 1.0;
    } else {
      r += 100.0;
    }
    if (dl == 0) r += 100.0;
    else r += log10(100.0 / dl) * 5.0;
  }
  return r;
}

__device__ inline double reward_dev(Ctx &X, int a, bool moved, bool engage, int n_hit) {
  return reward_core(X.P, X.S, X.c, X.lane, X.E, X.env, a, moved, engage, n_hit);
}

__device__ __forceinline__ void reset_env_dev(const KParams &P, const KState &S, int env, Rng &rng) {
  const long long E = P.E;
  double duct = 1.0 + rng.beta13();
  S.duct[env] = duct;
  bool box = P.box_hi[0] > P.box_lo[0] && P.box_hi[1] > P.box_lo[1];
  unsigned long long box_ctr = ((unsigned long long)(uint32_t)S.envi[7 * E + env]) << 32;
  for (int a = 0; a < P.A; a++) {
    size_t ai = (size_t)a * E + env;
    int t = S.sp_types[a];
    int x, y;
    if (S.sp_pos_env) {
      x = S.sp_pos_env[((size_t)env * P.A + a) * 2];
      y = S.sp_pos_env[((size_t)env * P.A + a) * 2 + 1];
    } else {
      x = S.sp_pos[2 * a];
      y = S.sp_pos[2 * a + 1];
    }
    if (box) {
      for (int tries = 0; tries < 64; tries++) {
        uint32_t o[4];
        o[0] = (uint32_t)box_ctr;
        o[1] = (uint32_t)(box_ctr >> 32);
        o[2] = rng.g0;
        o[3] = rng.g1 ^ 0x80000000u;
        philox10(o, rng.k0 ^ 0x5bd1e995u, rng.k1);
        box_ctr++;
        int bx = P.box_lo[0] + (int)(o[0] % (uint32_t)(P.box_hi[0] - P.box_lo[0]));
        int by = P.box_lo[1] + (int)(o[1] % (uint32_t)(P.box_hi[1] - P.box_lo[1]));
        if (!(cell_bits(S.mask2, P.W16, bx, by) & 1u)) { x = bx; y = by; break; }
      }
    }
    if (S.sp_randls[a]) {
      x = rng.randint(98, 99);
      y = rng.randint(48, 56);
    }
    S.pos[ai] = pack_pos(x, y);
    S.radar[ai] = 1;
    S.miss[ai] = (uint8_t)missiles0(t);
    S.mkind[ai] = K_PYINT;
    S.alive[ai] = 1;
    S.type[ai] = (uint8_t)t;
    S.steps[ai] = 0;
    S.tl_cnt[ai] = 0;
    double dl = 0.0;
    if (t == T_LS) {
      int dx = x - P.lz_x, dy = y - P.lz_y;
      dl = sqrt((double)(dx * dx + dy * dy));
    }
    S.dist_lz[ai] = dl;
  }
  S.envi[0 * E + env] = P.nb;
  S.envi[1 * E + env] = P.nr;
  S.envi[2 * E + env] = 0;
  S.envi[3 * E + env] = 0;
  S.envi[4 * E + env] = 0;
  S.envi[7 * E + env] = S.envi[7 * E + env] + 1;
}

__device__ inline Rng make_rng(const KParams &P, const KState &S, int env) {
  Rng r;
  r.mode = P.rng_mode;
  r.k0 = (uint32_t)P.seed;
  r.k1 = (uint32_t)(P.seed >> 32);
  unsigned long long gid = (unsigned long long)(P.env_base + env);
  r.g0 = (uint32_t)gid;
  r.g1 = (uint32_t)(gid >> 32);
  r.ctr = S.rng[env];
  r.err = 0;
  r.tape = S.tape;
  if (P.rng_mode == 1 && S.tape_off) {
    r.tape_lo = S.tape_off[env];
    r.tape_hi = S.tape_off[env + 1];
  } else {
    r.tape_lo = r.tape_hi = 0;
  }
  return r;
}

__device__ __forceinline__ void build_row(const KParams &P, const KState &S, const Cols &c, const double *duct_col,
                          int el, int k, float *row, const float *xg, bool only_observed) {
  const int side = k >= P.nb;
  const int own0 = side ? P.nb : 0;
  const int ns = side ? P.nr : P.nb;
  const int kl = k - own0;
  const int D = side_D(P, side);
  const int G = P.G;
  if (!c.alive0[k * PADB + el] || (only_observed && !c.obsd[k * PADB + el])) {
    for (int d = 0; d < D; d++) row[d] = 0.0f;
    return;
  }
  const int tk = c.type[k * PADB + el];
  const uint32_t p = c.pos_cur[k * PAD + el];
  const int px = pos_x(p), py = pos_y(p);
  int idx;
  if (tk == T_LS || tk == T_MEDIUM) {
    const f32x4 *w = (const f32x4 *)(S.winf + ((size_t)win_cls(tk) * G * G + (size_t)(px * G + py)) * 52);
    f32x4 v[7];
#pragma unroll
    for (int q = 0; q < 7; q++) v[q] = w[q];
    f32x4 *r4 = (f32x4 *)row;
#pragma unroll
    for (int q = 0; q < 6; q++) r4[q] = v[q];
    row[24] = v[6].x;
    idx = 25;
  } else {
    const f32x4 *w = (const f32x4 *)(S.winf + (size_t)(px * G + py) * 52);
    f32x4 v[13];
#pragma unroll
    for (int q = 0; q < 13; q++) v[q] = w[q];
    f32x4 *r4 = (f32x4 *)row;
#pragma unroll
    for (int q = 0; q < 12; q++) r4[q] = v[q];
    row[48] = v[12].x;
    idx = 49;
  }
  row[idx++] = xg[px];
  row[idx++] = xg[py];
  row[idx++] = (float)c.radar_cur[k * PAD + el];
  row[idx++] = (float)c.miss_cur[k * PADB + el] * (tk == T_SMALL ? 0.25f : 0.125f);
  for (int il = 0; il < ns; il++) {
    if (il == kl) continue;
    const int i = own0 + il;
    if (c.alive0[i * PADB + el]) {
      const bool nw = il < kl;
      const uint32_t q = nw ? c.pos_cur[i * PAD + el] : c.pos_old[i * PAD + el];
      row[idx] = xg[pos_x(q)];
      row[idx + 1] = xg[pos_y(q)];
      row[idx + 2] = (float)(nw ? c.radar_cur[i * PAD + el] : c.radar_old[i * PAD + el]);
      const int m = nw ? c.miss_cur[i * PADB + el] : c.miss_old[i * PADB + el];
      row[idx + 3] = (float)m * (c.type[i * PADB + el] == T_SMALL ? 0.25f : 0.125f);
    } else {
      row[idx] = row[idx + 1] = row[idx + 2] = row[idx + 3] = 0.0f;
    }
    idx += 4;
  }
  row[idx++] = (float)c.tcnt[k * PAD + el];
  row[idx++] = tk == T_LS ? 1.0f : 0.0f;
  row[idx++] = (float)(duct_col[el] / 2.0);
  for (; idx < D; idx++) row[idx] = 0.0f;
}

__device__ inline void copy_side(const float *stage, float *out, int ns, int D, int ne, long long genv0,
                                 long long stride = 0) {
  if (!out) return;
  const int lane = threadIdx.x & (WAVE - 1);
  const int S4 = stage_stride(ns) >> 2;
  const int D4 = D >> 2;
  const int n4 = ne * ns * D4;
  const f32x4 *st4 = (const f32x4 *)stage;
  if (stride && stride != (long long)ns * D) {
    const int per = ns * D4;
    for (int i = lane; i < n4; i += WAVE) {
      const int e = i / per, q = i - e * per, r = e * ns + q / D4;
      ((f32x4 *)(out + (genv0 + e) * stride))[q] = st4[r * S4 + (q - (q / D4) * D4)];
    }
    return;
  }
// ... 745 lines not shown
          for (int a = 0; a < A; a++) {
            if (a < nb) COLW(c.reward, a) = COLW(c.reward, a) - COLW(c.reward, a);
            else COLW(c.reward, a) += 100.0;
          }
          ev[3] += 1;
        }
      }
    }
  }
  ev[2] = ev[2] + 1;
  if (nbp > 0 && nrp > 0) {
    double bx = (double)bsx / nbp, by = (double)bsy / nbp, rx = (double)rsx / nrp, ry = (double)rsy / nrp;
    cog = sqrt((bx - rx) * (bx - rx) + (by - ry) * (by - ry));
  }
  *cog_p = cog;
  return done;
}

__device__ __forceinline__ bool env_resets(const KParams &P, int done, int steps_env) {
  return P.auto_reset && (done == 0 || (P.episode_steps > 0 && steps_env >= P.episode_steps));
}

__device__ __forceinline__ void env_tail(const KParams &P, const KState &S, Cols &c, int lane, int env,
                                         int nb, int A, const Neut &N, int (&ev)[8],
                                         const int (&hits)[2], int nbp, int nrp, int bsx, int bsy,
                                         int rsx, int rsy, Rng &rng, float *rew_b, float *rew_r,
                                         int32_t *done_out, float *cog_out, bool quiet = false) {
  const long long E = P.E;
  const int nr = A - nb;
  double cog;
  const int done = env_tail_core(P, c, lane, nb, A, N, ev, hits, nbp, nrp, bsx, bsy, rsx, rsy, &cog, quiet);
  const int steps_env = ev[2];
  if (P.rew_f64) {
    for (int a = 0; a < nb; a++)
      if (rew_b) ((double *)rew_b)[(size_t)env * nb + a] = COLW(c.reward, a);
    for (int a = 0; a < nr; a++)
      if (rew_r) ((double *)rew_r)[(size_t)env * nr + a] = COLW(c.reward, nb + a);
    if (cog_out) ((double *)cog_out)[env] = cog;
  } else {
    for (int a = 0; a < nb; a++)
      if (rew_b) rew_b[(size_t)env * nb + a] = (float)COLW(c.reward, a);
    for (int a = 0; a < nr; a++)
      if (rew_r) rew_r[(size_t)env * nr + a] = (float)COLW(c.reward, nb + a);
    if (cog_out) cog_out[env] = (float)cog;
  }
  if (done_out) done_out[env] = done;
  prof_stamp(S, 2);
  const bool do_reset = env_resets(P, done, steps_env);
  for (int a = 0; a < A; a++) {
    size_t ai = (size_t)a * E + env;
    int side = a >= nb;
    bool killed = (N.mask[side] >> (a - (side ? nb : 0))) & 1u;
    S.pos[ai] = COLW(c.pos_cur, a);
    S.radar[ai] = COLW(c.radar_cur, a);
    S.steps[ai] = COLW(c.steps, a);
    if (quiet) continue;
    S.miss[ai] = COLB(c.miss_cur, a);
    S.mkind[ai] = COLB(c.mkind, a);
    S.alive[ai] = COLB(c.alive0, a) && !killed;
    S.tl_cnt[ai] = (uint16_t)COLW(c.tcnt, a);
  }
  if (quiet) {
    S.envi[2 * E + env] = ev[2];
    if (done == 0) {
      S.envi[3 * E + env] = ev[3];
      S.envi[4 * E + env] = ev[4];
    }
  } else {
#pragma unroll
    for (int q = 0; q < 8; q++) S.envi[q * E + env] = ev[q];
  }
  if (do_reset) reset_env_dev(P, S, env, rng);
  if (!quiet || !P.trained_red || do_reset) S.rng[env] = rng.ctr;
  if (rng.err) S.err[env] |= rng.err;
}

#include "lnw_quiet.inc"

extern __shared__ __attribute__((aligned(16))) char lds_dyn[];

template <int NB, int NR, bool CW, bool REFW, int UN, bool PS, bool SL>
__device__ __forceinline__ void step_body(
    const KParams &P, KState S, void *actions, const uint8_t *row_kind, float *obs_b, float *obs_r,
    float *rew_b, float *rew_r, int32_t *done_out, float *cog_out) {
  static_assert(UN == 1 || (NB > 0 && EPW == WAVE && !REFW), "units need the two-wave templated kernel");
  const int unit = UN > 1 ? (int)(threadIdx.x / (2 * WAVE)) : 0;
  const int lane = threadIdx.x & (WAVE - 1);
  const int wid = UN > 1 ? (int)((threadIdx.x / WAVE) & 1) : (int)(threadIdx.x / WAVE);
  const int epw = P.epw;
  const int env0 = (UN > 1 ? blockIdx.x * UN + unit : xcd_chunk(P, (int)blockIdx.x, (int)gridDim.x)) * epw;
  if (UN > 1 && S.prof) S.prof += (size_t)(blockIdx.x * (UN - 1) + unit) * PROF_SLOTS;
  const int env = env0 + lane;
  const long long E = P.E;
  const bool valid = lane < epw && env < E;
  const int nenv = (E - env0) < epw ? (int)(E - env0) : epw;
  constexpr bool ST = NB > 0;
  const int nb = ST ? NB : P.nb, nr = ST ? NR : P.nr;
  const int A = nb + nr;
  const int qbig_rows = !(ST && NB == NR && EPW == WAVE && P.los_mode == 0) ? 0
                        : SL ? (P.qdirect ? WAVE : 0)
                             : (epw * NB <= WAVE ? epw * NB : 0);
  LdsLayout L = lds_layout(A, nb, nr, S.nmax, P.G * P.W16, P.G, qbig_rows);
  const int lstride = (L.total + 15) & ~15;
  Cols c = carve(lds_dyn + unit * lstride, L);
  __shared__ double duct_all[UN][WAVE];
  __shared__ int prog_all[UN], qclaim_all[UN];
  __shared__ int r2_all[UN][WAVE];
  __shared__ int ushare[2];
  double *duct_col = duct_all[unit];
  int &prog = prog_all[unit], &qclaim = qclaim_all[unit];
  int *r2col = r2_all[unit];
  if (UN > 1 && threadIdx.x == 0) { ushare[0] = 0; ushare[1] = 0; }
  const bool psplit = PS && CW && NB == 4 && NR == 4 && UN == 1 && EPW == WAVE && P.los_mode == 0 &&
                      !(P.dbg_skip & 515) && !(P.dbg_skip & 16384);
  const bool emit = ST && P.los_mode != 1 && nenv == WAVE && !(P.dbg_skip & 3) && !P.no_obs && !psplit;
  constexpr int NW = ST && EPW == WAVE ? 2 : 1;
  if (NW == 1 && wid == 1) return;
  constexpr int MAXPRE = 4;
  const int dt = P.act_dtype;
  const bool pre = ST && NW == 2 && dt == LNW_ACT_F32 && !(P.dbg_skip & 4) && !(P.dbg_skip & 8388608);
  f32x4 vpre[MAXPRE];
  if (pre) preload_rows_f32<NW, MAXPRE>(actions, env0, nenv, A, wid, vpre);
  int evp[8] = {0, 0, 0, 0, 0, 0, 0, 0};
  Rng rngp{};
  const bool evpre = ST && !CW && NW == 2 && UN == 1 && NB == NR && epw * NB <= WAVE && P.los_mode == 0 &&
                     !(P.dbg_skip & (1 << 29));
  if (evpre && wid == 0 && valid) {
#pragma unroll
    for (int q = 0; q < 8; q++) evp[q] = S.envi[q * E + env];
    rngp = make_rng(P, S, env);
  }
  if (wid == 0) {
    prof_stamp(S, 0);
    prof_put(S, 30, (unsigned long long)__builtin_amdgcn_s_getreg((3 << 11) | 20));
    prof_put(S, 31, (unsigned long long)__builtin_amdgcn_s_getreg((31 << 11) | 4));
  } else if (wid == 1) {
    prof_put(S, 29, (unsigned long long)__builtin_amdgcn_s_getreg((31 << 11) | 4));
  }

  stage_mask<NW>(P, S, c.mask, (int)threadIdx.x - unit * NW * WAVE);
  const uint32_t *mask = c.mask;
  load_state<NB + NR, NW>(P, S, c, lane, env, valid, wid);
  double duct = valid ? S.duct[env] : 1.0;
  if (wid == 0) {
    duct_col[lane] = duct;
    r2col[lane] = max_range2(P, duct);
    if (lane == 0) prog = -1;
  }
  __syncthreads();
  if (wid == 0) prof_stamp(S, 4);

  bool pend = false;
  if (!(P.dbg_skip & 4)) {
    if (pre)
      pend = move_phase_pre<NW, MAXPRE>(P, S, c, actions, row_kind, mask, env0, nenv, A, wid, vpre);
    else if (dt == LNW_ACT_F32)
      pend = move_phase<LNW_ACT_F32, NW>(P, S, c, actions, row_kind, mask, env0, nenv, A, wid);
    else if (dt == LNW_ACT_F64)
      pend = move_phase<LNW_ACT_F64, NW>(P, S, c, actions, row_kind, mask, env0, nenv, A, wid);
    else
      pend = move_phase<LNW_ACT_I32, NW>(P, S, c, actions, row_kind, mask, env0, nenv, A, wid);
  }
  const bool qcap = ST && P.los_mode == 0 && !(P.dbg_skip & 3) && !(P.dbg_skip & 512);
  const bool astar = NW > 1 ? __syncthreads_or(pend) != 0 : true;
  if constexpr (ST && NW > 1) {
    if (qcap) {
      if (wid == 0) prof_stamp(S, 6);
      if (astar) {
        if (wid == 0) move_astar_pass(P, S, c, nenv, A);
        __syncthreads();
      }
      if (wid == 0) prof_stamp(S, 7);
      bool wq;
      if (NB == NR && UN == 1 && P.epw * NB <= WAVE && !(P.dbg_skip & 268435456))
        wq = wg_quiet_spread_t<NB, NB>(P, c, lane, r2col);
      else
        wq = __all(env_quiet_t<NB, NR>(P, c, lane, r2col[lane]));
      if (wid == 0) prof_stamp(S, 8);
#ifdef LNW_DIAG
      if (P.dbg_skip & (1 << 24)) {
        wq = __all(env_quiet_t<NB, NR>(P, c, lane, r2col[lane] + (P.dbg_skip >> 30)));
        if (wid == 0) prof_stamp(S, 12);
      }
#endif
      if (__builtin_expect(wq, 1)) {
        if constexpr (UN > 1)
          quiet_step_units_t<NB, NR, UN>(P, S, c, lds_dyn, L, lstride, unit, lane, env, wid, duct_all,
                                         ushare, actions, obs_b, obs_r, rew_b, rew_r, done_out, cog_out,
                                         env0, valid);
        else
          quiet_step_t<NB, NR, SL>(P, S, c, lane, env, wid, duct_col, &qclaim, actions, obs_b, obs_r, rew_b,
                               rew_r, done_out, cog_out, env0, nenv, valid, evpre, evp, rngp);
        return;
      }
      if (UN > 1) __syncthreads();
    }
  }
#ifdef LNW_PROBE_QUIET_ONLY
  if constexpr (ST && NW > 1) return;
#endif
  const bool phase_o = !((P.dbg_skip & 1) || emit || P.no_obs);
  if (wid == 1 && !psplit) {
    if constexpr (ST) {
      if (emit) emit_wave_t<NB>(P, S, c, duct_col, &prog, obs_b, obs_r, env0);
    }
    prof_stamp(S, 5);
    return;
  }
  if (!qcap && astar && !(P.dbg_skip & 4)) {
    move_astar_pass(P, S, c, nenv, A);
    wave_lds_sync();
  }

  prof_stamp(S, 1);
  if (valid && !(P.dbg_skip & 2)) {
    if (emit) publish_progress(&prog, 0);
// ... 256 lines not shown
            thr_v = (double)rintf((float)engagement * (float)COLB(c.miss_cur, a));
          else
            thr_v = rint(engagement * (double)COLB(c.miss_cur, a));
          if (!isfinite(thr_v)) { X.rng.err |= LNW_ERRF_NAN_ROUND; thr_v = 0.0; }
          engage = thr_v > 0.0;
          int tn = (int)COLW(c.tcnt, a);
          if (engage && tn > 0 && !(P.dbg_skip & 65536)) {
            const uint16_t *tl = S.tl + (size_t)a * P.T * E + env;
            if constexpr (CW) {
              for (int q0 = 0; q0 < tn; q0 += 8) {
                uint64_t pk0 = 0, pk1 = 0;
#pragma unroll
                for (int u = 0; u < 8; u++) {
                  const uint64_t v = q0 + u < tn ? (uint64_t)tl[(size_t)(q0 + u) * E] : 0ull;
                  if (u < 4) pk0 |= v << (16 * u);
                  else pk1 |= v << (16 * (u - 4));
                }
                const int nq = tn - q0 < 8 ? tn - q0 : 8;
                for (int u = 0; u < nq; u++) {
                  const uint16_t tg = (uint16_t)((u < 4 ? pk0 : pk1) >> (16 * (u & 3)));
                  if (fire_dev(X, a, tg & 0xff, tg >> 8, engagement, keng, N)) destroyed++;
                }
              }
            } else {
              uint16_t nx = tl[0];
              for (int q = 0; q < tn; q++) {
                const uint16_t tg = nx;
                if (q + 1 < tn) nx = tl[(size_t)(q + 1) * E];
                if (fire_dev(X, a, tg & 0xff, tg >> 8, engagement, keng, N)) destroyed++;
              }
            }
          }
          if (side) ev[6] += destroyed; else ev[5] += destroyed;
          if (!isfinite(a0)) { X.rng.err |= LNW_ERRF_NAN_ROUND; COLW(c.radar_cur, a) = 0; }
          else {
            double rr = rint(a0);
            COLW(c.radar_cur, a) = (int)fmin(fmax(rr, -2147483648.0), 2147483647.0);
          }
          uint32_t pn = COLW(c.pos_new, a);
          moved = (pn & 0x80000000u) != 0;
          if (moved) COLW(c.pos_cur, a) = pn & 0x7fffffffu;
        }
        tp[0] += prof_now(S) - t0;
        t0 = prof_now(S);
        if (al && !(P.dbg_skip & 128)) {
          if constexpr (REFW) march_pairs_ref(X, a);
          if constexpr (ST) {
            if (!side) get_obs_t<NB, NR, CW>(X, a, 0, NB);
            else get_obs_t<NR, NB, CW>(X, a, NB, 0);
          } else {
            get_obs_dev(X, a);
          }
        }
        tp[2] += prof_now(S) - t0;
        t0 = prof_now(S);
        double r = 0.0;
        if (al && !(P.dbg_skip & 256)) r = reward_dev(X, a, moved, engage, destroyed);
        COLW(c.reward, a) = r;
        if (al) {
          if (!side) {
            if (P.side_blue ? destroyed > 0 : engage) COLB(c.eng, a) = 1;
          } else {
            if (!P.trained_red ? engage : destroyed > 1) COLB(c.eng, a) = 1;
          }
          hits[side] += destroyed;
        }
        tp[3] += prof_now(S) - t0;
        if (emit) publish_progress(&prog, a + 1);
        if (a < 8) prof_stamp(S, 6 + a);
      }
    }
    env_tail(P, S, c, lane, env, nb, A, N, ev, hits, nbp, nrp, bsx, bsy, rsx, rsy, X.rng, rew_b,
             rew_r, done_out, cog_out);
    if (S.prof && lane == 0)
      for (int q = 0; q < 4; q++) prof_put(S, 16 + q, tp[q]);
  }
  prof_stamp(S, 3);
  if (!phase_o) return;
  __syncthreads();
  if constexpr (ST) write_obs_t<NB, NR>(P, S, c, duct_col, obs_b, obs_r, env0, nenv);
  else write_obs(P, S, c, duct_col, obs_b, obs_r, env0, nenv, false);
}

template <int NB, int NR, bool CW = false, bool REFW = false, int UN = 1, bool PS = false, bool SL = false>
__global__ __launch_bounds__(NB > 0 && EPW == WAVE ? 2 * WAVE * UN : WAVE, NB > 0 ? 2 : 1) void step_kernel(
    KParams P, KState S, void *actions, const uint8_t *row_kind, float *obs_b, float *obs_r,
    float *rew_b, float *rew_r, int32_t *done_out, float *cog_out) {
  step_body<NB, NR, CW, REFW, UN, PS, SL>(P, S, actions, row_kind, obs_b, obs_r, rew_b, rew_r, done_out, cog_out);
}

#include "lnw_group.inc"

template <int NB = 0, int NR = 0, bool CW = false>
__global__ __launch_bounds__(NB > 0 && CW ? 2 * WAVE : WAVE) void observe_kernel(KParams P, KState S, int sel,
                                                                                 float *obs_b, float *obs_r) {
  constexpr int NW = NB > 0 && CW ? 2 : 1;
  const int lane = threadIdx.x & (WAVE - 1);
  const int wid = NW > 1 ? (int)(threadIdx.x / WAVE) : 0;
  const int epw = P.epw;
  const int env0 = xcd_chunk(P, (int)blockIdx.x, (int)gridDim.x) * epw;
  const int env = env0 + lane;
  const long long E = P.E;
  const bool valid = lane < epw && env < E;
  const int nenv = (E - env0) < epw ? (int)(E - env0) : epw;
  const int A = P.A, nb = P.nb;
  LdsLayout L = lds_layout(A, P.nb, P.nr, S.nmax, P.G * P.W16, P.G);
  Cols c = carve(lds_dyn, L);
  __shared__ double duct_col[WAVE];
  __shared__ unsigned long long ctr1[NW > 1 ? WAVE : 1];
  __shared__ uint32_t err1[NW > 1 ? WAVE : 1];
  for (int w = (int)threadIdx.x; w < P.G * P.W16; w += NW * WAVE) c.mask[w] = S.mask2[w];
  const uint32_t *mask = c.mask;
  load_state<NB + NR, NW>(P, S, c, lane, env, valid, wid);
  double duct = valid ? S.duct[env] : 1.0;
  if (wid == 0) duct_col[lane] = duct;
  __syncthreads();
  int a0 = 0, a1 = A;
  if (sel >= 0) { a0 = sel; a1 = sel + 1; }
  else if (sel == LNW_OBS_BLUE) { a1 = nb; }
  else if (sel == LNW_OBS_RED) { a0 = nb; }
  const bool split = NW > 1 && sel == LNW_OBS_ALL;
  int wa0 = a0, wa1 = a1;
  if (NW > 1) {
    if (split) { wa0 = wid ? nb : 0; wa1 = wid ? A : nb; }
    else if (wid == 1) { wa1 = wa0; }
  }
  unsigned long long fctr = 0;
  uint32_t ferr = 0;
  if (valid) {
    Cols cw = c;
    if (NW > 1 && wid == 1) cw.observed = (uint32_t *)(lds_dyn + L.act0);
    Ctx X{P, S, cw, lane, env, duct_col, make_rng(P, S, env), mask, E, max_range2(P, duct),
          S.envi[2 * E + env]};
    if constexpr (NB > 0 && CW) {
      pair_tables_t<NB, NR, false>(X);
      if (split && wid == 1) {
        long long nd = 0;
        for (int a = 0; a < nb; a++) {
          if (!COLB(c.alive0, a)) continue;
          uint32_t pp[NR], am, fb, bm;
          mask_walk_t<NB, NR>(X, a, 0, NB, pp, am, fb, bm);
          nd += __builtin_popcount(bm);
        }
        if (X.rng.mode == 1) {
          const long long len = X.rng.tape_hi - X.rng.tape_lo, cur = (long long)X.rng.ctr;
          X.rng.ctr = (unsigned long long)(cur + nd <= len ? cur + nd : (cur > len ? cur : len));
        } else {
          X.rng.ctr += (unsigned long long)nd;
        }
      }
    } else if constexpr (NB > 0) {
      if (P.los_mode != 1) los_prefetch_t<NB, NR>(X);
    }
    for (int a = wa0; a < wa1; a++) {
      if (!COLB(c.alive0, a)) continue;
      if constexpr (NB > 0) {
        if (a < NB) get_obs_t<NB, NR, CW>(X, a, 0, NB);
        else get_obs_t<NR, NB, CW>(X, a, NB, 0);
      } else {
        if (P.los_mode == 2) march_pairs_ref(X, a);
        get_obs_dev(X, a);
      }
      COLB(c.obsd, a) = 1;
      S.tl_cnt[(size_t)a * E + env] = (uint16_t)COLW(c.tcnt, a);
    }
    fctr = X.rng.ctr;
    ferr = X.rng.err;
    if (NW > 1 && wid == 1) {
      ctr1[lane] = split ? fctr : 0ull;
      err1[lane] = ferr;
    }
// ... 204 lines not shown
  int t = types[i];
  int sx = pos[2 * i], sy = pos[2 * i + 1];
  int nx, ny;
  bool fin = move_target_dev(sx, sy, ship_speed(t), act[2 * i], act[2 * i + 1],
                             is_f32[i] ? K_F32 : K_F64, nx, ny);
  rounded[2 * i] = nx;
  rounded[2 * i + 1] = ny;
  bool f = fin && can_move_to_h(P, S, nx, ny) &&
           check_path_h(P, S, t, sx, sy, nx, ny, open + threadIdx.x, WAVE);
  ok[i] = f ? 1 : 0;
}

__global__ __launch_bounds__(64) void path_query_kernel(KParams P, KState S, const int8_t *types,
                                                        const int16_t *st, const int16_t *tg,
                                                        long long n, uint8_t *out) {
  __shared__ uint32_t open[OPEN_CAP * WAVE];
  long long i = (long long)blockIdx.x * WAVE + threadIdx.x;
  if (i >= n) return;
  out[i] = check_path_h(P, S, types[i], st[2 * i], st[2 * i + 1], tg[2 * i], tg[2 * i + 1],
                        open + threadIdx.x, WAVE) ? 1 : 0;
}

__global__ void los_query_kernel(KParams P, KState S, const int16_t *pairs, long long n,
                                 uint8_t *out) {
  long long i = (long long)blockIdx.x * blockDim.x + threadIdx.x;
  if (i >= n) return;
  out[i] = (uint8_t)los_q(P, S, S.mask2, pairs[4 * i], pairs[4 * i + 1], pairs[4 * i + 2],
                          pairs[4 * i + 3]);
}

__global__ void fill_uniform_kernel(float *out, long long n, unsigned long long seed,
                                    unsigned long long offset) {
  long long i = (long long)blockIdx.x * blockDim.x + threadIdx.x;
  long long base = i * 4;
  if (base >= n) return;
  float u[4];
  philox_u4(seed, (offset >> 2) + (unsigned long long)i, u);
#pragma unroll
  for (int k = 0; k < 4; k++)
    if (base + k < n) out[base + k] = u[k];
}

thread_local std::string g_err;

int fail(int code, const std::string &msg) {
  g_err = msg;
  return code;
}

#define HIPCHK(expr)                                                                  \
  do {                                                                                \
    hipError_t _e = (expr);                                                           \
    if (_e != hipSuccess)                                                             \
      return fail(LNW_EDEVICE, std::string(#expr) + ": " + hipGetErrorString(_e));    \
  } while (0)

void host_constants(KParams &k) {
  const double base = std::sqrt((4.0 / 3.0) * 6370.0 * 2.0);
  const int masts[2] = {15, 30};
  for (int i = 0; i < 2; i++)
    for (int j = 0; j < 2; j++) {
      double d = base * (std::sqrt((double)masts[i] / 1000.0) + std::sqrt((double)masts[j] / 1000.0));
      k.d5[i][j] = d / 5.0;
    }
  for (int i = 0; i < 2; i++)
    k.den[i] = (base * (std::sqrt((double)masts[i] / 1000.0) + std::sqrt(15.0 / 1000.0))) / 5.0;
  k.det_q[0] = 0.345 - 0.1;
  k.det_q[1] = 0.345 + 0.1;
  const double ps[2] = {0.45, 0.63};
  for (int h = 0; h < 2; h++)
    for (int n = 0; n < 9; n++) {
      k.hit64[h][n] = 1.0 - std::pow(1.0 - ps[h], (double)n);
      float pn = powf((float)(1.0 - ps[h]), (float)n);
      k.hit32[h][n] = 1.0f - pn;
    }
}

}

struct lnw_handle {
  int device = 0;
  lnw_params params{};
  KParams kp{};
  int E = 0, nb = 0, nr = 0, A = 0, T = 0, nmax = 0;
  long long env_base = 0;
  int G = 0, W16 = 0;
  bool terrain = false;
  uint8_t *d_grid = nullptr;
  float *d_gridf = nullptr, *d_winf = nullptr, *d_dummy = nullptr;
  unsigned long long *d_prof = nullptr;
  size_t prof_cap = 0;
  lnw_analytics ana{};
  unsigned long long *ctr = nullptr;
  int dbg_skip = 0;
  bool prof = false, force_generic = false, no_group = false, group_fits = false, no_units = false;
  bool no_slab = false;
  bool force_group = false;
  bool no_split_rows = false;
  bool store_wt = false;
  bool units_fit = false;
  bool contact = false;
  int last_kernel = LNW_KERNEL_NONE;
  bool has_medium = false;
  unsigned long long terrain_hash = 0;
  uint32_t *d_mask2 = nullptr, *d_mvtab = nullptr, *d_lostab = nullptr;
  uint32_t *pos = nullptr;
  int32_t *radar = nullptr, *steps = nullptr, *envi = nullptr;
  uint8_t *miss = nullptr, *mkind = nullptr, *alive = nullptr, *type = nullptr;
  double *dist_lz = nullptr, *duct = nullptr, *bear_val = nullptr, *d_atan = nullptr;
  uint8_t *bear_ship = nullptr;
  uint16_t *tl_cnt = nullptr, *tl = nullptr;
  unsigned long long *rng = nullptr;
  uint32_t *err = nullptr;
  int32_t *sp_types = nullptr, *sp_pos = nullptr, *sp_randls = nullptr, *sp_pos_env = nullptr;
  bool sp_pos_env_on = false;
  const double *tape = nullptr;
  const long long *tape_off = nullptr;
  std::vector<void *> allocs;
};

namespace {

template <class T>
int dalloc(lnw_handle *h, T **p, size_t n) {
  void *q = nullptr;
  hipError_t e = hipMalloc(&q, n * sizeof(T) + 16);
  if (e != hipSuccess) return fail(LNW_ENOMEM, std::string("hipMalloc: ") + hipGetErrorString(e));
  (void)hipMemset(q, 0, n * sizeof(T) + 16);
  h->allocs.push_back(q);
  *p = (T *)q;
  return 0;
}

KState make_state(lnw_handle *h) {
  KState s{};
  s.pos = h->pos; s.radar = h->radar; s.miss = h->miss; s.mkind = h->mkind; s.alive = h->alive;
  s.type = h->type; s.steps = h->steps; s.dist_lz = h->dist_lz; s.tl_cnt = h->tl_cnt; s.tl = h->tl;
  s.duct = h->duct; s.envi = h->envi; s.rng = h->rng; s.err = h->err;
  s.bear_val = h->bear_val; s.bear_ship = h->bear_ship; s.atan_deg = h->d_atan;
  s.grid = h->d_grid; s.gridf = h->d_gridf; s.winf = h->d_winf; s.dummy = h->d_dummy; s.prof = nullptr; s.ana = h->ana; s.ctr = h->ctr; s.mask2 = h->d_mask2; s.mvtab = h->d_mvtab; s.lostab = h->d_lostab;
  s.tape = h->tape; s.tape_off = h->tape_off;
  s.sp_types = h->sp_types; s.sp_pos = h->sp_pos; s.sp_randls = h->sp_randls;
  s.sp_pos_env = h->sp_pos_env_on ? h->sp_pos_env : nullptr;
  s.nmax = h->nmax;
  return s;
}

size_t step_lds_bytes(const lnw_handle *h) {
  LdsLayout L = lds_layout(h->A, h->nb, h->nr, h->nmax, h->G * h->W16, h->G);
  return (size_t)L.total;
}

int device_ncu(int dev) {
  static int cache[64] = {0};
  int &c = cache[dev & 63];
  if (c == 0) {
    int n = 0;
    c = hipDeviceGetAttribute(&n, hipDeviceAttributeMultiprocessorCount, dev) == hipSuccess && n > 0 ? n : 256;
  }
  return c;
}

bool step_qdirect(const lnw_handle *h, int epw) {
  const bool tmpl = !h->force_generic && !h->has_medium && h->params.los_mode == 0 && h->nb == h->nr &&
                    h->nb >= 2 && h->nb <= 4 && EPW == WAVE;
  if (!tmpl) return false;
  if (epw * h->nb <= WAVE) return true;
  if (h->nb != 4 || h->contact || h->no_slab || epw * h->nb > 2 * WAVE) return false;
  const LdsLayout L = lds_layout(h->A, h->nb, h->nr, h->nmax, h->G * h->W16, h->G, WAVE);
  int per_cu = (int)((160 * 1024) / ((size_t)L.total + 1024));
  if (per_cu > 4) per_cu = 4;
  return (h->E + epw - 1) / epw <= (long long)device_ncu(h->device) * per_cu;
}

size_t step_launch_lds_bytes(const lnw_handle *h, int epw) {
  const int rows = step_qdirect(h, epw) ? (epw * h->nb < WAVE ? epw * h->nb : WAVE) : 0;
  LdsLayout L = lds_layout(h->A, h->nb, h->nr, h->nmax, h->G * h->W16, h->G, rows);
  return (size_t)L.total;
}

int choose_epw(const lnw_handle *h) {
  if (const char *e = getenv("LNW_EPW_RT")) {
    int v = atoi(e);
    if (v >= 1 && v <= EPW) return v;
  }
  int ncu = 256;
  hipDeviceProp_t prop;
  if (hipGetDeviceProperties(&prop, h->device) == hipSuccess && prop.multiProcessorCount > 0)
    ncu = prop.multiProcessorCount;
  const bool two_wave = !h->force_generic && h->params.los_mode != 2 && h->nb == h->nr && h->nb >= 2 && h->nb <= 4 && EPW == WAVE;
  const int by_waves = two_wave ? 4 : 8;
  auto slots = [&](int e) {
    const size_t lds = step_launch_lds_bytes(h, e) + 1024;
    int per_cu = (int)((160 * 1024) / lds);
    if (per_cu > by_waves) per_cu = by_waves;
    if (per_cu < 1) per_cu = 1;
    return (long long)ncu * per_cu;
  };
  const int min_epw = two_wave ? 16 : 1;
  int epw = EPW;
  while (epw > min_epw && (h->E + epw - 1) / epw < slots(epw)) epw /= 2;
  if ((h->E + epw - 1) / epw > slots(epw) && epw < EPW) epw *= 2;
  return epw;
}

}

void prof_report(lnw_handle *h, hipStream_t st, int nwg) {
  std::vector<unsigned long long> t((size_t)nwg * PROF_SLOTS);
  if (hipMemcpyAsync(t.data(), h->d_prof, t.size() * 8, hipMemcpyDeviceToHost, st) != hipSuccess ||
      hipStreamSynchronize(st) != hipSuccess)
    return;
  double sL = 0, sM = 0, sS = 0, sW = 0, s1 = 0, sa[8] = {0}, sq[4] = {0}, sp[4] = {0}, sg[4] = {0},
         st3[3] = {0, 0, 0};
  int nq = 0;
  unsigned long long t0 = ~0ull, tend0 = 0, tend1 = 0;
  int n1 = 0;
  for (int w = 0; w < nwg; w++) {
    const unsigned long long *r = &t[(size_t)w * PROF_SLOTS];
    sL += (double)(r[4] - r[0]);
    sM += (double)(r[1] - r[4]);
    sS += (double)(r[2] - r[1]);
    sW += (double)(r[3] - r[2]);
    if (r[5]) { s1 += (double)(r[5] - r[0]); n1++; if (r[5] > tend1) tend1 = r[5]; }
    for (int q = 0; q < 4; q++) sp[q] += (double)r[16 + q];
    for (int q = 0; q < 4; q++) sg[q] += (double)r[20 + q];
    if (r[14]) {
      nq++;
// ... 81 lines not shown
      se[x] += e; nx[x]++;
      if (e > mx[x]) mx[x] = e;
    }
    {
      std::vector<std::pair<int, double>> v;
      for (int w = 0; w < nwg; w++) {
        const unsigned long long *r = &t[(size_t)w * PROF_SLOTS];
        if (!r[5] || r[5] < t0) continue;
        v.push_back({(int)((r[30] & 15) << 8 | ((r[31] >> 8) & 0xff)), (double)(r[5] - t0) * us});
      }
      std::sort(v.begin(), v.end());
      std::vector<double> means, spans;
      for (size_t i = 0; i < v.size();) {
        size_t j = i;
        double sm = 0, lo = 1e30, hi = -1e30;
        while (j < v.size() && v[j].first == v[i].first) { sm += v[j].second; lo = std::min(lo, v[j].second); hi = std::max(hi, v[j].second); j++; }
        means.push_back(sm / (double)(j - i));
        spans.push_back(hi - lo);
        i = j;
      }
      std::sort(means.begin(), means.end());
      std::sort(spans.begin(), spans.end());
      if (!means.empty())
        fprintf(stderr, "[lnw prof] CUs %zu: CU-mean wave-1 end p10 %.1f p50 %.1f p90 %.1f max %.1f; within-CU span p50 %.1f p90 %.1f max %.1f us\n",
                means.size(), means[means.size() / 10], means[means.size() / 2], means[means.size() * 9 / 10], means.back(),
                spans[spans.size() / 2], spans[spans.size() * 9 / 10], spans.back());
    }
    {
      std::vector<int> key(nwg);
      for (int w = 0; w < nwg; w++) {
        const unsigned long long *r = &t[(size_t)w * PROF_SLOTS];
        key[w] = (int)((r[30] & 15) << 12 | ((r[31] >> 8) & 0xff) << 4 | ((r[31] >> 4) & 3));
      }
      std::vector<int> sk = key;
      std::sort(sk.begin(), sk.end());
      double e0[2] = {0, 0}, m0[2] = {0, 0};
      int n0[2] = {0, 0}, same = 0;
      for (int w = 0; w < nwg; w++) {
        const unsigned long long *r = &t[(size_t)w * PROF_SLOTS];
        const int cnt = (int)(std::upper_bound(sk.begin(), sk.end(), key[w]) - std::lower_bound(sk.begin(), sk.end(), key[w]));
        const int k = cnt > 1 ? 1 : 0;
        if (r[3] < t0) continue;
        const double e = (double)(r[3] - t0) * us;
        e0[k] += e; n0[k]++;
        if (e > m0[k]) m0[k] = e;
        same += ((r[31] >> 4) & 3) == ((r[29] >> 4) & 3);
      }
      fprintf(stderr, "[lnw prof] wave-0 SIMD: alone %d (end mean %.1f max %.1f us), shared %d (mean %.1f max %.1f us); "
                      "waves 0/1 on one SIMD in %d workgroups\n",
              n0[0], n0[0] ? e0[0] / n0[0] : 0.0, m0[0], n0[1], n0[1] ? e0[1] / n0[1] : 0.0, m0[1], same);
    }
    fprintf(stderr, "[lnw prof] wave-1 end by XCC (n/mean/max us):");
    for (int x = 0; x < 16; x++)
      if (nx[x]) fprintf(stderr, " %d:%d/%.1f/%.1f", x, nx[x], se[x] / nx[x], mx[x]);
    fprintf(stderr, "; block%%8==xcc for %d of %d\n",
            [&] { int k = 0; for (int w = 0; w < nwg; w++) k += (int)(t[(size_t)w * PROF_SLOTS + 30] & 15) == (w & 7); return k; }(), nwg);
  }
  {
    double rq = 0;
    int nr2 = 0;
    for (int w = 0; w < nwg; w++) {
      const unsigned long long *r = &t[(size_t)w * PROF_SLOTS];
      if (r[14] && r[12] > r[8] && r[8]) { rq += (double)(r[12] - r[8]); nr2++; }
    }
    if (nr2) fprintf(stderr, "[lnw prof] repeated quiet test (diagnostics): %.2f us\n", rq / nr2 * us);
  }
  {
    double q0 = 0, q1 = 0, rb = 0, rc = 0;
    int nd = 0;
    for (int w = 0; w < nwg; w++) {
      const unsigned long long *r = &t[(size_t)w * PROF_SLOTS];
      if (!r[14] || !r[28] || !r[15] || !r[27] || r[28] < r[9]) continue;
      nd++;
      q0 += (double)(r[27] - r[8]);
      q1 += (double)(r[15] - r[8]);
      rb += (double)(r[28] - r[9]);
      rc += (double)(r[5] - r[28]);
    }
    if (nd)
      fprintf(stderr, "[lnw prof] quiet direct %d: phase-Q work wave 0 %.2f, wave 1 %.2f us; after the barrier "
                      "rows staged %.2f, stored %.2f us\n",
              nd, q0 / nd * us, q1 / nd * us, rb / nd * us, rc / nd * us);
  }
  if (nq)
    fprintf(stderr, "[lnw prof] quiet workgroups %d: M %.2f us, A*+barrier %.2f us, quiet test %.2f us, Q+barrier %.2f us; "
                    "tail: rewards %.2f, cog %.2f, env_tail+outputs %.2f us\n",
            nq, sq[0] / nq * us, sq[1] / nq * us, sq[2] / nq * us, sq[3] / nq * us, st3[0] / nq * us,
            st3[1] / nq * us, st3[2] / nq * us);
  const int ns = nwg - nq;
  fprintf(stderr, "[lnw prof] phase S workgroups %d, per agent (us):", ns);
  for (int a = 0; a < 8; a++) fprintf(stderr, " %.2f", ns ? sa[a] / ns * us : 0.0);
  fprintf(stderr, "; section totals take_action %.2f, LOS prefetch %.2f, get_obs %.2f, reward %.2f us\n",
          ns ? sp[0] / ns * us : 0.0, ns ? sp[1] / ns * us : 0.0, ns ? sp[2] / ns * us : 0.0,
          ns ? sp[3] / ns * us : 0.0);
  fprintf(stderr, "[lnw prof] get_obs parts (templated): pair walk %.2f, observed stores %.2f, bearings+fixes %.2f, fix targets %.2f us\n",
          ns ? sg[0] / ns * us : 0.0, ns ? sg[1] / ns * us : 0.0, ns ? sg[2] / ns * us : 0.0,
          ns ? sg[3] / ns * us : 0.0);
}

extern "C" {

int lnw_abi_version(void) { return LNW_ABI_VERSION; }
const char *lnw_last_error(void) { return g_err.c_str(); }

int lnw_set_analytics(lnw_handle *h, const lnw_analytics *a) {
  if (!h) return fail(LNW_EINVAL, "null handle");
  if (!a) { h->ana = lnw_analytics{}; return 0; }
  if ((a->eng_log && (!a->eng_count || a->eng_cap < 0)) || (a->ew_log && (!a->ew_count || a->ew_cap < 0)))
    return fail(LNW_EINVAL, "analytics log without a counter or with a negative capacity");
  h->ana = *a;
  return 0;
}

int lnw_hit_tables(double *tab64, float *tab32) {
  KParams k{};
  host_constants(k);
  for (int h = 0; h < 2; h++)
    for (int n = 0; n < 9; n++) {
      if (tab64) tab64[h * 9 + n] = k.hit64[h][n];
      if (tab32) tab32[h * 9 + n] = k.hit32[h][n];
    }
  return 0;
}

int lnw_create(const lnw_params *params, int32_t n_envs, int32_t nb, int32_t nr, int32_t device,
               int64_t env_id_base, lnw_handle **out) {
  if (!params || !out) return fail(LNW_EINVAL, "null argument");
  if (n_envs <= 0) return fail(LNW_EINVAL, "n_envs must be > 0");
  if (nb < 1 || nr < 1 || nb > 16 || nr > 16)
    return fail(LNW_EUNSUPPORTED, "need 1 <= nb, nr <= 16 ships per side");
  HIPCHK(hipSetDevice(device));
  lnw_handle *h = new lnw_handle();
  h->device = device;
  if (const char *dbg = getenv("LNW_DEBUG_SKIP")) h->dbg_skip = atoi(dbg);
#ifndef LNW_DIAG
  constexpr int kResultPreserving = 512 | 32768 | 131072 | 4194304 | 8388608 | (1 << 28) | (1 << 29);
  if (h->dbg_skip & ~kResultPreserving) {
    const int bad = h->dbg_skip & ~kResultPreserving;
    delete h;
    return fail(LNW_EINVAL, "LNW_DEBUG_SKIP bits " + std::to_string(bad) +
                                " change results; they exist only in the diagnostics build (-DLNW_DIAG)");
  }
#endif
  h->prof = getenv("LNW_PROF") != nullptr;
  h->force_generic = getenv("LNW_FORCE_GENERIC") != nullptr;
  h->no_group = getenv("LNW_NO_GROUP") != nullptr;
  h->force_group = getenv("LNW_FORCE_GROUP") != nullptr;
  h->no_split_rows = getenv("LNW_NO_SPLIT_ROWS") != nullptr;
  h->no_units = getenv("LNW_NO_UNITS") != nullptr;
  h->no_slab = getenv("LNW_NO_SLAB") != nullptr;
  h->kp.xcd_remap = getenv("LNW_NO_XCD_REMAP") == nullptr ? 1 : 0;
  h->kp.group_march = getenv("LNW_GROUP_MARCH") != nullptr ? 1 : 0;
  {
    const int ns = nb > nr ? nb : nr;
    const double side_bytes = (double)n_envs * ns * (4 * ns + 52) * 4.0;
    h->store_wt = getenv("LNW_NO_STORE_WT") == nullptr && side_bytes < 2147483648.0;
  }
  h->params = *params;
  h->E = n_envs; h->nb = nb; h->nr = nr; h->A = nb + nr;
  h->nmax = nb > nr ? nb : nr;
  h->T = h->nmax + h->nmax * h->nmax;
  h->env_base = env_id_base;
  const size_t E = (size_t)n_envs, A = (size_t)h->A;
  int rc = 0;
  rc |= dalloc(h, &h->pos, A * E);
  rc |= dalloc(h, &h->radar, A * E);
  rc |= dalloc(h, &h->miss, A * E);
  rc |= dalloc(h, &h->mkind, A * E);
  rc |= dalloc(h, &h->alive, A * E);
  rc |= dalloc(h, &h->type, A * E);
  rc |= dalloc(h, &h->steps, A * E);
  rc |= dalloc(h, &h->dist_lz, A * E);
  rc |= dalloc(h, &h->tl_cnt, A * E);
  rc |= dalloc(h, &h->tl, A * (size_t)h->T * E);
  rc |= dalloc(h, &h->duct, E);
  rc |= dalloc(h, &h->envi, 8 * E);
  rc |= dalloc(h, &h->rng, E);
  rc |= dalloc(h, &h->err, E);
  rc |= dalloc(h, &h->bear_val, (size_t)h->nmax * h->nmax * E);
  rc |= dalloc(h, &h->bear_ship, (size_t)h->nmax * h->nmax * E);
  rc |= dalloc(h, &h->sp_types, 64);
  rc |= dalloc(h, &h->sp_pos, 128);
  rc |= dalloc(h, &h->sp_randls, 64);
  rc |= dalloc(h, &h->d_dummy, 4 * 64);
  rc |= dalloc(h, &h->d_atan, (size_t)LOS_W * LOS_W);
  if (rc) {
    std::string m = g_err;
    lnw_destroy(h);
    return fail(LNW_ENOMEM, m);
  }
  {
    std::vector<double> at((size_t)LOS_W * LOS_W);
    for (int dy = -R_LOS; dy <= R_LOS; dy++)
      for (int dx = -R_LOS; dx <= R_LOS; dx++)
// ... 72 lines not shown
    for (int x = 0; x < G; x++)
      for (int y = 0; y < G; y++) {
        float *w7 = &wf[((size_t)x * G + y) * 52];
        for (int i = 0; i < 7; i++)
          for (int j = 0; j < 7; j++) w7[i * 7 + j] = cellv(x - 3 + i, y - 3 + j);
        float *w5 = &wf[((size_t)G * G + (size_t)x * G + y) * 52];
        for (int i = 0; i < 5; i++)
          for (int j = 0; j < 5; j++) w5[i * 5 + j] = cellv(x - 1 + i, y - 1 + j);
        float *wm = &wf[((size_t)2 * G * G + (size_t)x * G + y) * 52];
        for (int i = 0; i < 5; i++)
          for (int j = 0; j < 5; j++) wm[i * 5 + j] = cellv(x - 2 + i, y - 2 + j);
      }
    HIPCHK(hipMemcpy(h->d_winf, wf.data(), wf.size() * sizeof(float), hipMemcpyHostToDevice));
  }
  KParams &k = h->kp;
  k.G = G;
  k.W16 = h->W16;
  int n = G * h->W16;
  build_mask_kernel<<<(n + 255) / 256, 256>>>(h->d_grid, G, h->W16, k.move_thr, k.ew_thr, h->d_mask2);
  HIPCHK(hipGetLastError());
  long long nm = (long long)MV_CLASSES * G * G * MV_W * MV_W;
  build_move_table_kernel<<<(unsigned)((nm + WAVE - 1) / WAVE), WAVE>>>(h->d_mask2, G, h->W16, h->d_mvtab);
  HIPCHK(hipGetLastError());
  long long nl = (long long)G * G * LOS_W;
  const int mwords = G * h->W16 * 4 <= 64 * 1024 ? G * h->W16 : 0;
  {
    int ncu = 256;
    hipDeviceProp_t prop;
    if (hipGetDeviceProperties(&prop, h->device) == hipSuccess && prop.multiProcessorCount > 0)
      ncu = prop.multiProcessorCount;
    const long long need = (nl + 255) / 256, cap = (long long)ncu * 8;
    build_los_table_kernel<<<(unsigned)(need < cap ? need : cap), 256, (size_t)mwords * 4>>>(
        h->d_mask2, G, h->W16, h->d_lostab, mwords);
  }
  HIPCHK(hipGetLastError());
  HIPCHK(hipDeviceSynchronize());
  h->terrain = true;
  {
    const size_t need = step_launch_lds_bytes(h, WAVE / h->nb);
    if (need > (size_t)GROUP_LDS_MAX) return fail(LNW_EUNSUPPORTED, "agent count needs more LDS than a CU has");
    const LdsLayout GLy = lds_layout(h->A, h->nb, h->nr, h->nmax, h->G * h->W16, h->G);
    const size_t gneed = (size_t)group_lds(GLy, h->G * h->W16, h->A, h->nb * h->nr, h->kp.atan_odd != 0).total + 1024;
    h->group_fits = group_lds(GLy, h->G * h->W16, h->A, h->nb * h->nr, h->kp.atan_odd != 0).ms >= 0;
    static unsigned long long lds_opt_in = 0;
    const unsigned long long dbit = 1ull << (h->device & 63);
    const size_t uneed = (size_t)UNITS * ((step_lds_bytes(h) + 15) & ~(size_t)15);
    h->units_fit = uneed <= (size_t)UNITS_LDS_MAX;
    if (!(lds_opt_in & dbit) && (need > 64 * 1024 || gneed > 64 * 1024 || uneed > 64 * 1024)) {
      HIPCHK(hipFuncSetAttribute((const void *)step_kernel<4, 4, false, false, 1, false, true>,
                                 hipFuncAttributeMaxDynamicSharedMemorySize, GROUP_LDS_MAX));
      const void *ks[17] = {(const void *)step_kernel<4, 4, true, false, 1, true>,
                            (const void *)step_kernel<0, 0>,       (const void *)step_kernel<2, 2>,
                            (const void *)step_kernel<3, 3>,       (const void *)step_kernel<4, 4>,
                            (const void *)step_kernel<2, 2, true>, (const void *)step_kernel<3, 3, true>,
                            (const void *)step_kernel<4, 4, true>, (const void *)step_kernel<0, 0, false, true>,
                            (const void *)observe_kernel<0, 0, false>, (const void *)step_group_kernel,
                            (const void *)observe_kernel<2, 2, false>, (const void *)observe_kernel<3, 3, false>,
                            (const void *)observe_kernel<4, 4, false>, (const void *)observe_kernel<2, 2, true>,
                            (const void *)observe_kernel<3, 3, true>, (const void *)observe_kernel<4, 4, true>};
      for (const void *kk : ks)
        HIPCHK(hipFuncSetAttribute(kk, hipFuncAttributeMaxDynamicSharedMemorySize, GROUP_LDS_MAX));
      HIPCHK(hipFuncSetAttribute((const void *)step_kernel<4, 4, false, false, UNITS>,
                                 hipFuncAttributeMaxDynamicSharedMemorySize, UNITS_LDS_MAX));
      lds_opt_in |= dbit;
    }
  }
  (void)hipGetLastError();
  h->kp.epw = choose_epw(h);
  return 0;
}

int lnw_set_rng(lnw_handle *h, int32_t mode, uint64_t seed, const double *tape_dev,
                const int64_t *tape_off_dev) {
  if (!h) return fail(LNW_EINVAL, "null handle");
  if (mode != LNW_RNG_PHILOX && mode != LNW_RNG_TAPE) return fail(LNW_EINVAL, "bad rng mode");
  if (mode == LNW_RNG_TAPE && (!tape_dev || !tape_off_dev))
    return fail(LNW_EINVAL, "tape mode needs tape and offsets");
  HIPCHK(hipSetDevice(h->device));
  h->kp.rng_mode = mode;
  h->kp.seed = seed;
  h->tape = tape_dev;
  h->tape_off = (const long long *)tape_off_dev;
  HIPCHK(hipMemset(h->rng, 0, sizeof(unsigned long long) * h->E));
  return 0;
}

static int apply_side_types(lnw_handle *h, const int32_t *types, bool apply) {
  int nmed[2] = {0, 0};
  for (int a = 0; a < h->A; a++) {
    const int t = types[a];
    if (t != LNW_SMALL && t != LNW_LARGE && t != LNW_LS && t != LNW_MEDIUM)
      return fail(LNW_EUNSUPPORTED, "ship type must be small, large, ls or medium");
    if (t == LNW_MEDIUM) nmed[a >= h->nb]++;
    if (h->params.discrete && t == LNW_LS)
      return fail(LNW_EUNSUPPORTED, "LandingShip has no value_to_coordinates (DISCRETE mode)");
  }
  for (int sd = 0; sd < 2; sd++) {
    const int ns = sd ? h->nr : h->nb;
    if (nmed[sd] && nmed[sd] != ns)
      return fail(LNW_EUNSUPPORTED, "medium ships need a side of medium ships only (the reference's "
                                    "rows are sized by the fastest ship, game.py:595-610)");
  }
  if (apply) {
    h->kp.wc[0] = nmed[0] ? 25 : 49;
    h->kp.wc[1] = nmed[1] ? 25 : 49;
    h->has_medium = nmed[0] || nmed[1];
  }
  return 0;
}

int lnw_reset(lnw_handle *h, const uint8_t *env_mask_dev, const lnw_spawn *spawn,
              const int32_t *pos_dev, void *stream) {
  if (!h || !spawn) return fail(LNW_EINVAL, "null argument");
  if (!h->terrain) return fail(LNW_ESTATE, "lnw_load_terrain must be called first");
  HIPCHK(hipSetDevice(h->device));
  if (int rc = apply_side_types(h, spawn->types, false)) return rc;
  for (int a = 0; a < h->A; a++)
    if (!spawn->rand_ls[a] && (spawn->pos[a][0] < 0 || spawn->pos[a][0] >= h->G ||
                               spawn->pos[a][1] < 0 || spawn->pos[a][1] >= h->G))
      return fail(LNW_EINVAL, "spawn position outside the grid");
  apply_side_types(h, spawn->types, true);
  hipStream_t st = (hipStream_t)stream;
  HIPCHK(hipMemcpy(h->sp_types, spawn->types, sizeof(int32_t) * h->A, hipMemcpyHostToDevice));
  HIPCHK(hipMemcpy(h->sp_pos, spawn->pos, sizeof(int32_t) * 2 * h->A, hipMemcpyHostToDevice));
  HIPCHK(hipMemcpy(h->sp_randls, spawn->rand_ls, sizeof(int32_t) * h->A, hipMemcpyHostToDevice));
  h->kp.box_lo[0] = spawn->box_lo[0]; h->kp.box_lo[1] = spawn->box_lo[1];
  h->kp.box_hi[0] = spawn->box_hi[0]; h->kp.box_hi[1] = spawn->box_hi[1];
  if (pos_dev) {
    const size_t n = (size_t)h->E * h->A * 2;
    if (!h->sp_pos_env && dalloc(h, &h->sp_pos_env, n)) return LNW_ENOMEM;
    HIPCHK(hipMemcpyAsync(h->sp_pos_env, pos_dev, n * sizeof(int32_t), hipMemcpyDeviceToDevice, st));
  }
  h->sp_pos_env_on = pos_dev != nullptr;
  KState s = make_state(h);
  reset_kernel<<<(h->E + 255) / 256, 256, 0, st>>>(h->kp, s, env_mask_dev);
  HIPCHK(hipGetLastError());
  return 0;
}

namespace {
int step_launch(lnw_handle *h, void *actions_dev, int32_t action_dtype,
                const uint8_t *row_kind_dev, float *obs_blue_dev, float *obs_red_dev, float *rew_blue_dev,
                float *rew_red_dev, int32_t *done_dev, float *cog_dev, void *stream) {
  if (!h || !actions_dev) return fail(LNW_EINVAL, "null argument");
  if (!h->terrain) return fail(LNW_ESTATE, "lnw_load_terrain must be called first");
  if (action_dtype != LNW_ACT_F32 && action_dtype != LNW_ACT_F64 && action_dtype != LNW_ACT_I32)
    return fail(LNW_EINVAL, "bad action dtype");
  if (action_dtype == LNW_ACT_I32 && !h->params.discrete)
    return fail(LNW_EINVAL, "integer actions go with DISCRETE mode only");
  if (action_dtype == LNW_ACT_F32 && h->params.discrete)
    return fail(LNW_EINVAL, "DISCRETE mode takes int32 (ndarray) or float64 (list rows) actions");
  if ((obs_blue_dev == nullptr) != (obs_red_dev == nullptr))
    return fail(LNW_EINVAL, "observation outputs: both or neither");
  KParams k = h->kp;
  k.act_dtype = action_dtype;
  k.no_obs = obs_blue_dev == nullptr ? 1 : 0;
  k.dbg_skip = h->dbg_skip;
  k.store_wt = h->store_wt;
  KState s = make_state(h);
  k.qdirect = step_qdirect(h, k.epw) ? 1 : 0;
  size_t lds = step_launch_lds_bytes(h, k.epw);
  dim3 grid((h->E + k.epw - 1) / k.epw), block(WAVE);
  hipStream_t st = (hipStream_t)stream;
  bool generic = h->force_generic;
  const bool templated = k.los_mode != 2 && !generic && !h->has_medium && h->nb == h->nr && h->nb >= 2 && h->nb <= 4 &&
                         !(h->force_group && h->group_fits);
  const bool use_group = k.los_mode != 2 && !templated && !generic && !h->no_group && h->group_fits;
  const bool units = templated && h->nb == 4 && !h->contact && !h->no_units && h->units_fit && k.epw == EPW &&
                     k.los_mode == 0 && h->E % (EPW * UNITS) == 0 && !(h->dbg_skip & (1 | 2 | 512));
  const unsigned nwg = use_group ? (unsigned)((h->E + GEPW - 1) / GEPW) : grid.x;
  if (h->prof) {
    const size_t slots = (size_t)nwg * PROF_SLOTS;
    if (slots > h->prof_cap) {
      HIPCHK(hipStreamSynchronize(st));
      if (h->d_prof) { (void)hipFree(h->d_prof); h->d_prof = nullptr; h->prof_cap = 0; }
      HIPCHK(hipMalloc(&h->d_prof, slots * sizeof(unsigned long long)));
      h->prof_cap = slots;
    }
    HIPCHK(hipMemsetAsync(h->d_prof, 0, slots * sizeof(unsigned long long), st));
    s.prof = h->d_prof;
  }
#define LNW_STEP(NB_, NR_, CW_, RW_)                                                             \
  step_kernel<NB_, NR_, CW_, RW_><<<grid, dim3(NB_ > 0 && EPW == WAVE ? 2 * WAVE : WAVE), lds, st>>>(k, s, actions_dev, row_kind_dev, obs_blue_dev, \
                                                 obs_red_dev, rew_blue_dev, rew_red_dev,        \
                                                 done_dev, cog_dev)
  const bool cw = h->contact;
  h->last_kernel = units ? LNW_KERNEL_UNITS
                   : k.los_mode == 2 ? LNW_KERNEL_REFLOS
                   : templated ? (cw ? LNW_KERNEL_TEAM_CONTACT : LNW_KERNEL_TEAM)
                   : use_group ? LNW_KERNEL_GROUP : LNW_KERNEL_GENERIC;
  if (units) {
    step_kernel<4, 4, false, false, UNITS><<<dim3(h->E / (EPW * UNITS)), dim3(2 * WAVE * UNITS),
                                             (size_t)UNITS * ((lds + 15) & ~(size_t)15), st>>>(
        k, s, actions_dev, row_kind_dev, obs_blue_dev, obs_red_dev, rew_blue_dev, rew_red_dev, done_dev,
        cog_dev);
  }
  else if (k.los_mode == 2) LNW_STEP(0, 0, false, true);
  else if (templated && h->nb == 4) {
    if (cw && k.los_mode == 0 && (k.no_obs || !h->no_split_rows))
      step_kernel<4, 4, true, false, 1, true><<<grid, dim3(2 * WAVE), lds, st>>>(
          k, s, actions_dev, row_kind_dev, obs_blue_dev, obs_red_dev, rew_blue_dev, rew_red_dev, done_dev, cog_dev);
    else if (cw) LNW_STEP(4, 4, true, false);
    else if (k.qdirect && k.epw * 4 > WAVE)
      step_kernel<4, 4, false, false, 1, false, true><<<grid, dim3(2 * WAVE), lds, st>>>(
          k, s, actions_dev, row_kind_dev, obs_blue_dev, obs_red_dev, rew_blue_dev, rew_red_dev, done_dev, cog_dev);
    else LNW_STEP(4, 4, false, false);
  }
  else if (templated && h->nb == 3) { if (cw) LNW_STEP(3, 3, true, false); else LNW_STEP(3, 3, false, false); }
  else if (templated && h->nb == 2) { if (cw) LNW_STEP(2, 2, true, false); else LNW_STEP(2, 2, false, false); }
  else if (use_group) {
    const GroupLds gl = group_lds(lds_layout(h->A, h->nb, h->nr, h->nmax, h->G * h->W16, h->G), h->G * h->W16,
                                  h->A, h->nb * h->nr, k.atan_odd != 0);
    const size_t glds = (size_t)gl.total;
    if (s.prof)
      fprintf(stderr, "[lnw prof] group kernel LDS %zu B (staged: target lists %d, dist_lz %d, bearing half table %d, pooled slopes %d)\n",
              glds, (int)(gl.tls >= 0), (int)(gl.dlz >= 0), (int)(gl.atab >= 0), (int)(gl.ms >= 0));
    step_group_kernel<<<dim3((h->E + GEPW - 1) / GEPW), dim3(GEPW * GL), glds, st>>>(
        k, s, actions_dev, row_kind_dev, obs_blue_dev, obs_red_dev, rew_blue_dev, rew_red_dev,
        done_dev, cog_dev);
  }
  else LNW_STEP(0, 0, false, false);
#undef LNW_STEP
  HIPCHK(hipGetLastError());
  if (s.prof) prof_report(h, st, (int)nwg);
  return 0;
}
}

int lnw_step(lnw_handle *h, void *actions_dev, int32_t action_dtype, const uint8_t *row_kind_dev,
             float *obs_blue_dev, float *obs_red_dev, float *rew_blue_dev, float *rew_red_dev,
             int32_t *done_dev, float *cog_dev, void *stream) {
  return step_launch(h, actions_dev, action_dtype, row_kind_dev, obs_blue_dev, obs_red_dev, rew_blue_dev,
                     rew_red_dev, done_dev, cog_dev, stream);
}

int lnw_step_seq(lnw_handle *h, const lnw_seq *seq, void *actions_dev, int32_t action_dtype,
                 const uint8_t *row_kind_dev, float *obs_blue_dev, float *obs_red_dev, float *rew_blue_dev,
                 float *rew_red_dev, int32_t *done_dev, float *cog_dev, void *stream) {
  if (!h || !seq) return fail(LNW_EINVAL, "null argument");
  if (seq->steps < 1) return fail(LNW_EINVAL, "seq->steps must be >= 1");
  if (seq->act_step < 0 || seq->kind_step < 0 || seq->obs_blue_step < 0 || seq->obs_red_step < 0 ||
      seq->rew_blue_step < 0 || seq->rew_red_step < 0 || seq->done_step < 0 || seq->cog_step < 0)
    return fail(LNW_EINVAL, "negative step stride");
  const long long asz = action_dtype == LNW_ACT_F64 ? 8 : 4, rsz = h->kp.rew_f64 ? 8 : 4;
  for (int k = 0; k < seq->steps; k++) {
    auto adv = [&](const void *p, long long stride, long long sz) {
      return p ? (void *)((char *)p + (long long)k * stride * sz) : nullptr;
    };
    if (int e = step_launch(h, adv(actions_dev, seq->act_step, asz), action_dtype,
                            (const uint8_t *)adv(row_kind_dev, seq->kind_step, 1),
                            (float *)adv(obs_blue_dev, seq->obs_blue_step, 4),
                            (float *)adv(obs_red_dev, seq->obs_red_step, 4),
                            (float *)adv(rew_blue_dev, seq->rew_blue_step, rsz),
                            (float *)adv(rew_red_dev, seq->rew_red_step, rsz),
                            (int32_t *)adv(done_dev, seq->done_step, 4), (float *)adv(cog_dev, seq->cog_step, rsz),
                            stream))
      return e;
  }
  return 0;
}

int lnw_observe(lnw_handle *h, int32_t agent, float *obs_blue_dev, float *obs_red_dev, void *stream) {
  return lnw_observe_ex(h, agent, obs_blue_dev, 0, obs_red_dev, 0, stream);
}

int lnw_observe_ex(lnw_handle *h, int32_t agent, float *obs_blue_dev, int64_t blue_env_stride,
                   float *obs_red_dev, int64_t red_env_stride, void *stream) {
  if (!h) return fail(LNW_EINVAL, "null handle");
  if (!h->terrain) return fail(LNW_ESTATE, "lnw_load_terrain must be called first");
  if (agent >= h->A || agent < LNW_OBS_RED) return fail(LNW_EINVAL, "bad agent selector");
  const int64_t row_b = (int64_t)h->nb * side_D(h->kp, 0), row_r = (int64_t)h->nr * side_D(h->kp, 1);
  if (blue_env_stride < 0 || red_env_stride < 0 || (blue_env_stride && (blue_env_stride < row_b || blue_env_stride % 4)) ||
      (red_env_stride && (red_env_stride < row_r || red_env_stride % 4)))
    return fail(LNW_EINVAL, "env stride: 0, or a multiple of 4 floats of at least the side's n * D");
  if (((uintptr_t)obs_blue_dev | (uintptr_t)obs_red_dev) & 15) return fail(LNW_EINVAL, "rows must be 16-B aligned");
  KState s = make_state(h);
  size_t lds = step_lds_bytes(h);
  dim3 grid((h->E + h->kp.epw - 1) / h->kp.epw), block(WAVE);
  hipStream_t st = (hipStream_t)stream;
  const bool tmpl = !h->force_generic && !h->has_medium && h->params.los_mode != 2 && h->nb == h->nr;
  const bool cw = h->contact;
  KParams k = h->kp;
  k.obs_stride[0] = blue_env_stride;
  k.obs_stride[1] = red_env_stride;
#define LNW_OBS(NB_, CW_)                                                                          \
  observe_kernel<NB_, NB_, CW_><<<grid, dim3(NB_ > 0 && CW_ ? 2 * WAVE : WAVE), lds, st>>>(k, s, agent, \
                                                                                    obs_blue_dev, obs_red_dev)
  if (tmpl && h->nb == 4) { if (cw) LNW_OBS(4, true); else LNW_OBS(4, false); }
  else if (tmpl && h->nb == 3) { if (cw) LNW_OBS(3, true); else LNW_OBS(3, false); }
  else if (tmpl && h->nb == 2) { if (cw) LNW_OBS(2, true); else LNW_OBS(2, false); }
  else LNW_OBS(0, false);
#undef LNW_OBS
  HIPCHK(hipGetLastError());
  return 0;
}

int lnw_state_field(lnw_handle *h, int32_t field, void **dev_ptr, int64_t *nbytes) {
  if (!h || !dev_ptr || !nbytes) return fail(LNW_EINVAL, "null argument");
  const int64_t E = h->E, A = h->A;
  switch (field) {
    case LNW_F_POS: *dev_ptr = h->pos; *nbytes = 4 * A * E; break;
    case LNW_F_RADAR: *dev_ptr = h->radar; *nbytes = 4 * A * E; break;
    case LNW_F_MISSILES: *dev_ptr = h->miss; *nbytes = A * E; break;
    case LNW_F_MKIND: *dev_ptr = h->mkind; *nbytes = A * E; break;
    case LNW_F_ALIVE: *dev_ptr = h->alive; *nbytes = A * E; break;
    case LNW_F_TYPE: *dev_ptr = h->type; *nbytes = A * E; break;
    case LNW_F_STEPS: *dev_ptr = h->steps; *nbytes = 4 * A * E; break;
    case LNW_F_DIST_LZ: *dev_ptr = h->dist_lz; *nbytes = 8 * A * E; break;
    case LNW_F_TL_CNT: *dev_ptr = h->tl_cnt; *nbytes = 2 * A * E; break;
    case LNW_F_TL: *dev_ptr = h->tl; *nbytes = 2 * A * h->T * E; break;
    case LNW_F_DUCT: *dev_ptr = h->duct; *nbytes = 8 * E; break;
    case LNW_F_ENV: *dev_ptr = h->envi; *nbytes = 4 * 8 * E; break;
    case LNW_F_RNG: *dev_ptr = h->rng; *nbytes = 8 * E; break;
    case LNW_F_ERR: *dev_ptr = h->err; *nbytes = 4 * E; break;
    default: return fail(LNW_EINVAL, "unknown state field");
  }
  return 0;
}

int lnw_tlist_cap(lnw_handle *h) { return h ? h->T : LNW_EINVAL; }

int lnw_step_kernel(lnw_handle *h) { return h ? h->last_kernel : LNW_EINVAL; }

namespace {
struct StateHeader {
  char magic[8];
  uint32_t version;
  int32_t E, nb, nr, T, G;
  int32_t rng_mode;
  int32_t pos_env_on;
  uint64_t seed;
  uint64_t terrain_hash;
  int64_t total;
  int32_t box_lo[2], box_hi[2];
  int32_t abi;
  uint8_t pad[128 - 8 - 4 - 7 * 4 - 3 * 8 - 4 * 4 - 4];
};
static_assert(sizeof(StateHeader) == 128, "state header is 128 bytes");

struct Section { void *dev; int64_t bytes; };

int state_sections(lnw_handle *h, std::vector<Section> &out) {
  out.clear();
  for (int f = 0; f < LNW_NFIELDS; f++) {
    void *p = nullptr;
    int64_t n = 0;
    if (int rc = lnw_state_field(h, f, &p, &n)) return rc;
    out.push_back({p, n});
  }
  out.push_back({h->sp_types, 64 * 4});
  out.push_back({h->sp_pos, 128 * 4});
  out.push_back({h->sp_randls, 64 * 4});
  out.push_back({h->sp_pos_env, (int64_t)h->E * h->A * 2 * 4});
  return 0;
}

inline int64_t sec_align(int64_t v) { return (v + 255) & ~(int64_t)255; }
}

// ... 4 lines not shown
  int64_t o = 256;
  for (const Section &x : s) o += sec_align(x.bytes);
  return o;
}

int lnw_get_state(lnw_handle *h, void *dst, int64_t nbytes, void *stream) {
  if (!h || !dst) return fail(LNW_EINVAL, "null argument");
  if (!h->terrain) return fail(LNW_ESTATE, "lnw_load_terrain must be called first");
  const int64_t total = lnw_state_bytes(h);
  if (nbytes < total) return fail(LNW_EINVAL, "snapshot buffer smaller than lnw_state_bytes()");
  HIPCHK(hipSetDevice(h->device));
  HIPCHK(hipStreamSynchronize((hipStream_t)stream));
  StateHeader hd;
  memset(&hd, 0, sizeof hd);
  memcpy(hd.magic, "LNWSTATE", 8);
  hd.version = 1;
  hd.E = h->E; hd.nb = h->nb; hd.nr = h->nr; hd.T = h->T; hd.G = h->G;
  hd.rng_mode = h->kp.rng_mode;
  hd.pos_env_on = h->sp_pos_env_on ? 1 : 0;
  hd.seed = h->kp.seed;
  hd.terrain_hash = h->terrain_hash;
  hd.total = total;
  for (int i = 0; i < 2; i++) { hd.box_lo[i] = h->kp.box_lo[i]; hd.box_hi[i] = h->kp.box_hi[i]; }
  hd.abi = LNW_ABI_VERSION;
  std::vector<Section> s;
  if (int rc = state_sections(h, s)) return rc;
  char *d = (char *)dst;
  char hbuf[256] = {0};
  memcpy(hbuf, &hd, sizeof hd);
  HIPCHK(hipMemcpy(d, hbuf, sizeof hbuf, hipMemcpyDefault));
  int64_t o = 256;
  for (const Section &x : s) {
    if (x.dev) {
      HIPCHK(hipMemcpy(d + o, x.dev, (size_t)x.bytes, hipMemcpyDefault));
    } else {
      const std::vector<char> z((size_t)x.bytes, 0);
      HIPCHK(hipMemcpy(d + o, z.data(), (size_t)x.bytes, hipMemcpyDefault));
    }
    o += sec_align(x.bytes);
  }
  return 0;
}

int lnw_set_state(lnw_handle *h, const void *src, int64_t nbytes, void *stream) {
  if (!h || !src) return fail(LNW_EINVAL, "null argument");
  if (!h->terrain) return fail(LNW_ESTATE, "lnw_load_terrain must be called first");
  HIPCHK(hipSetDevice(h->device));
  HIPCHK(hipStreamSynchronize((hipStream_t)stream));
  if (nbytes < (int64_t)sizeof(StateHeader)) return fail(LNW_EINVAL, "snapshot too short");
  StateHeader hd;
  HIPCHK(hipMemcpy(&hd, src, sizeof hd, hipMemcpyDefault));
  if (memcmp(hd.magic, "LNWSTATE", 8) != 0 || hd.version != 1)
    return fail(LNW_EINVAL, "not an lnw state snapshot (bad magic or version)");
  if (hd.abi != LNW_ABI_VERSION)
    return fail(LNW_EINVAL, "snapshot was taken by a library of another ABI version");
  const int64_t total = lnw_state_bytes(h);
  if (hd.E != h->E || hd.nb != h->nb || hd.nr != h->nr || hd.T != h->T || hd.G != h->G || hd.total != total)
    return fail(LNW_EINVAL, "snapshot shape (envs, team sizes, grid) differs from this handle");
  if (hd.terrain_hash != h->terrain_hash) return fail(LNW_EINVAL, "snapshot was taken on another terrain");
  if (nbytes < total) return fail(LNW_EINVAL, "snapshot shorter than its header says");
  if (hd.rng_mode == LNW_RNG_TAPE && (!h->tape || !h->tape_off))
    return fail(LNW_ESTATE, "snapshot is in tape mode: bind the tape (lnw_set_rng) before restoring");
  if (hd.pos_env_on && !h->sp_pos_env && dalloc(h, &h->sp_pos_env, (size_t)h->E * h->A * 2)) return LNW_ENOMEM;
  std::vector<Section> s;
  if (int rc = state_sections(h, s)) return rc;
  const char *p = (const char *)src;
  int32_t types[64];
  {
    int64_t ot = 256;
    for (int i = 0; i < LNW_NFIELDS; i++) ot += sec_align(s[i].bytes);
    HIPCHK(hipMemcpy(types, p + ot, sizeof types, hipMemcpyDefault));
    if (int rc = apply_side_types(h, types, false)) return rc;
  }
  int64_t o = 256;
  for (const Section &x : s) {
    if (x.dev) HIPCHK(hipMemcpy(x.dev, p + o, (size_t)x.bytes, hipMemcpyDefault));
    o += sec_align(x.bytes);
  }
  apply_side_types(h, types, true);
  h->kp.rng_mode = hd.rng_mode;
  if (hd.rng_mode == LNW_RNG_PHILOX) h->kp.seed = hd.seed;
  for (int i = 0; i < 2; i++) { h->kp.box_lo[i] = hd.box_lo[i]; h->kp.box_hi[i] = hd.box_hi[i]; }
  h->sp_pos_env_on = hd.pos_env_on != 0;
  return 0;
}

int lnw_set_counters(lnw_handle *h, uint64_t *counters_dev) {
  if (!h) return fail(LNW_EINVAL, "null handle");
  h->ctr = (unsigned long long *)counters_dev;
  return 0;
}

int lnw_set_reward_dtype(lnw_handle *h, int32_t f64) {
  if (!h) return fail(LNW_EINVAL, "null handle");
  h->kp.rew_f64 = f64 != 0;
  return 0;
}

int lnw_set_variant(lnw_handle *h, int32_t contact) {
  if (!h) return fail(LNW_EINVAL, "null handle");
  h->contact = contact != 0;
  return 0;
}

int lnw_set_epw(lnw_handle *h, int32_t epw) {
  if (!h) return fail(LNW_EINVAL, "null handle");
  if (epw < 0 || epw > EPW) return fail(LNW_EINVAL, "epw must be 0 (automatic) or 1..64");
  if (!h->terrain) return fail(LNW_ESTATE, "lnw_load_terrain must be called first");
  h->kp.epw = epw ? epw : choose_epw(h);
  return h->kp.epw;
}

int lnw_los_batch(const uint8_t *grid_dev, int32_t G, const int16_t *pairs_dev, int64_t n,
                  int32_t move_thr, int32_t ew_thr, uint8_t *out_dev, void *stream) {
  if (!grid_dev || !pairs_dev || !out_dev) return fail(LNW_EINVAL, "null argument");
  if (n <= 0) return 0;
  const size_t lds = (size_t)G * ((G + 15) / 16) * 4;
  if (lds <= 64 * 1024 && ((uintptr_t)pairs_dev & 7) == 0) {
    const long long per_block = (long long)(LB_THREADS / WAVE) * LB_RAYS_PER_WAVE;
    los_batch_kernel<<<(unsigned)((n + per_block - 1) / per_block), LB_THREADS, lds, (hipStream_t)stream>>>(
        grid_dev, G, pairs_dev, n, move_thr, ew_thr, out_dev);
  } else {
    los_batch_global_kernel<<<(unsigned)((n + 255) / 256), 256, 0, (hipStream_t)stream>>>(
        grid_dev, G, pairs_dev, n, move_thr, ew_thr, out_dev);
  }
  HIPCHK(hipGetLastError());
  return 0;
}

int lnw_astar_batch(const uint8_t *grid_dev, int32_t G, int32_t move_thr, const int8_t *types_dev,
                    const int16_t *start_dev, const int16_t *target_dev, int64_t n,
                    int16_t *plen_dev, int8_t *kind_dev, uint8_t *feasible_dev, void *stream) {
  if (!grid_dev || !types_dev || !start_dev || !target_dev || !plen_dev || !kind_dev || !feasible_dev)
    return fail(LNW_EINVAL, "null argument");
  if (n <= 0) return 0;
  astar_batch_kernel<<<(unsigned)((n + WAVE - 1) / WAVE), WAVE, 0, (hipStream_t)stream>>>(
      grid_dev, G, move_thr, types_dev, start_dev, target_dev, n, plen_dev, kind_dev, feasible_dev);
  HIPCHK(hipGetLastError());
  return 0;
}

int lnw_move_batch(lnw_handle *h, const int8_t *types_dev, const int16_t *pos_dev,
                   const double *act_dev, const uint8_t *is_f32_dev, int64_t n, int32_t *rounded_dev,
                   uint8_t *ok_dev, void *stream) {
  if (!h || !types_dev || !pos_dev || !act_dev || !is_f32_dev || !rounded_dev || !ok_dev)
    return fail(LNW_EINVAL, "null argument");
  if (!h->terrain) return fail(LNW_ESTATE, "lnw_load_terrain must be called first");
  if (n <= 0) return 0;
  KState s = make_state(h);
  move_batch_kernel<<<(unsigned)((n + WAVE - 1) / WAVE), WAVE, 0, (hipStream_t)stream>>>(
      h->kp, s, types_dev, pos_dev, act_dev, is_f32_dev, n, rounded_dev, ok_dev);
  HIPCHK(hipGetLastError());
  return 0;
}

int lnw_path_query(lnw_handle *h, const int8_t *types_dev, const int16_t *start_dev,
                   const int16_t *target_dev, int64_t n, uint8_t *out_dev, void *stream) {
  if (!h || !types_dev || !start_dev || !target_dev || !out_dev) return fail(LNW_EINVAL, "null argument");
  if (!h->terrain) return fail(LNW_ESTATE, "lnw_load_terrain must be called first");
  if (n <= 0) return 0;
  KState s = make_state(h);
  path_query_kernel<<<(unsigned)((n + WAVE - 1) / WAVE), WAVE, 0, (hipStream_t)stream>>>(
      h->kp, s, types_dev, start_dev, target_dev, n, out_dev);
  HIPCHK(hipGetLastError());
  return 0;
}

int lnw_los_query(lnw_handle *h, const int16_t *pairs_dev, int64_t n, uint8_t *out_dev, void *stream) {
  if (!h || !pairs_dev || !out_dev) return fail(LNW_EINVAL, "null argument");
  if (!h->terrain) return fail(LNW_ESTATE, "lnw_load_terrain must be called first");
  if (n <= 0) return 0;
  KState s = make_state(h);
  los_query_kernel<<<(unsigned)((n + 255) / 256), 256, 0, (hipStream_t)stream>>>(h->kp, s, pairs_dev, n, out_dev);
  HIPCHK(hipGetLastError());
  return 0;
}

int lnw_copy(void *dst, const void *src, int64_t nbytes, void *stream) {
  if (nbytes <= 0) return 0;
  if (!dst || !src) return fail(LNW_EINVAL, "null argument");
  HIPCHK(hipMemcpyAsync(dst, src, (size_t)nbytes, hipMemcpyDefault, (hipStream_t)stream));
  return 0;
}

int lnw_fill_uniform_f32(float *out_dev, int64_t n, uint64_t seed, uint64_t offset, void *stream) {
  if (!out_dev) return fail(LNW_EINVAL, "null argument");
  if (n <= 0) return 0;
  if (offset & 3) return fail(LNW_EINVAL, "offset must be a multiple of 4");
  long long nt = (n + 3) / 4;
  fill_uniform_kernel<<<(unsigned)((nt + 255) / 256), 256, 0, (hipStream_t)stream>>>(out_dev, n, seed, offset);
  HIPCHK(hipGetLastError());
  return 0;
}

}
```

Before: 1.624 billion env-steps/sec.

## Move rarely used state pointers to a device-side cold block and prefetch kernargs

Moves analytics, tape, spawn, bearing and counter pointers out of the by-value KState kernel argument into a device-resident KCold struct. The host deduplicates these blocks by byte comparison, so each launch passes only one pointer. This shrinks the kernel argument segment and adds an inline-asm prefetch that touches each 64-byte kernarg line at kernel entry. The cost is an extra dependent load wherever cold fields are read, including the bearing buffers on hot fix paths, plus small device allocations on configuration changes.

```diff
diff --git a/littoral-naval-warfare-marl_amd/csrc/lnw_device.h b/littoral-naval-warfare-marl_amd/csrc/lnw_device.h
--- a/littoral-naval-warfare-marl_amd/csrc/lnw_device.h
+++ b/littoral-naval-warfare-marl_amd/csrc/lnw_device.h
@@ -50,6 +50,22 @@
   int qdirect;
 };
 
+struct KCold {
+  lnw_analytics ana;
+  const double *tape;
+  const long long *tape_off;
+  const int32_t *sp_types;
+  const int32_t *sp_pos;
+  const int32_t *sp_randls;
+  const int32_t *sp_pos_env;
+  double *bear_val;
+  uint8_t *bear_ship;
+  unsigned long long *ctr;
+};
+static_assert(sizeof(KCold) == sizeof(lnw_analytics) + 9 * 8 && sizeof(lnw_analytics) == 72,
+              "KCold must have no implicit padding (blocks are compared bytewise)");
+typedef const KCold *ColdPtr;
+
 struct KState {
   uint32_t *pos;
   int32_t *radar;
@@ -65,25 +81,16 @@
   int32_t *envi;
   unsigned long long *rng;
   uint32_t *err;
-  double *bear_val;
-  uint8_t *bear_ship;
   const double *atan_deg;
   const uint8_t *grid;
   const float *gridf;
   const float *winf;
   float *dummy;
   unsigned long long *prof;
-  lnw_analytics ana;
-  unsigned long long *ctr;
+  ColdPtr cold;
   const uint32_t *mask2;
   const uint32_t *mvtab;
   const uint32_t *lostab;
-  const double *tape;
-  const long long *tape_off;
-  const int32_t *sp_types;
-  const int32_t *sp_pos;
-  const int32_t *sp_randls;
-  const int32_t *sp_pos_env;
   int nmax;
 };
 
diff --git a/littoral-naval-warfare-marl_amd/csrc/lnw_group.inc b/littoral-naval-warfare-marl_amd/csrc/lnw_group.inc
--- a/littoral-naval-warfare-marl_amd/csrc/lnw_group.inc
+++ b/littoral-naval-warfare-marl_amd/csrc/lnw_group.inc
@@ -362,7 +362,7 @@
   }
   GPROF_ADD(X, 5, tq);
   const uint32_t fixm = group_ballot(n >= 2, gsh);
-  if (S.ctr && n >= 2) X.pooled += (unsigned)n;
+  if (S.cold->ctr && n >= 2) X.pooled += (unsigned)n;
   if (fixm && !(P.dbg_skip & 16384)) {
     auto item = [&](int q) { return (uint32_t)((q < 4 ? it0 >> (16 * q) : it1 >> (16 * (q - 4))) & 0xffffu); };
     for (int q = 0; q < ni; q += 2) {
@@ -429,9 +429,9 @@
           err |= LNW_ERRF_NAN_ROUND;
         } else {
           const double rx = rint(mx), ry = rint(my);
-          if (S.ana.ew_log) {
+          if (S.cold->ana.ew_log) {
             const int ax = (int)fmin(fmax(rx, -32768.0), 32767.0), ay = (int)fmin(fmax(ry, -32768.0), 32767.0);
-            ana_record(S.ana.ew_log, S.ana.ew_count, S.ana.ew_cap, (uint32_t)(P.env_base + env),
+            ana_record(S.cold->ana.ew_log, S.cold->ana.ew_count, S.cold->ana.ew_cap, (uint32_t)(P.env_base + env),
                        (uint32_t)X.step | (uint32_t)side << 16, COLW(c.pos_cur, me),
                        (uint32_t)(uint16_t)ax | (uint32_t)(uint16_t)ay << 16);
           }
@@ -707,7 +707,7 @@
         if (engage && tn > 0 && !(P.dbg_skip & 65536)) {
           const uint16_t *tl = S.tl + (size_t)a * P.T * E + env;
           const int gsh = (int)(threadIdx.x & (WAVE - 1)) & ~(GL - 1);
-          const bool par = !S.ana.heatmap && !S.ana.coldmap && !S.ana.launch && !S.ana.eng_log &&
+          const bool par = !S.cold->ana.heatmap && !S.cold->ana.coldmap && !S.cold->ana.launch && !S.cold->ana.eng_log &&
                            !(P.dbg_skip & 32768);
           for (int q0 = 0; q0 < tn; q0 += GL) {
             const int q = q0 + sub;
@@ -753,7 +753,7 @@
     }
     env_tail(P, S, c, slot, env, nb, A, N, ev, hits, nbp, nrp, bsx, bsy, rsx, rsy, X.rng, rew_b,
              rew_r, done_out, cog_out);
-    if (S.ctr && X.pooled) atomicAdd(&S.ctr[3], (unsigned long long)X.pooled);
+    if (S.cold->ctr && X.pooled) atomicAdd(&S.cold->ctr[3], (unsigned long long)X.pooled);
     GPROF_ADD(X, 2, t0);
     GPROF_FLUSH(X);
   }
diff --git a/littoral-naval-warfare-marl_amd/csrc/lnw_kernels.hip b/littoral-naval-warfare-marl_amd/csrc/lnw_kernels.hip
--- a/littoral-naval-warfare-marl_amd/csrc/lnw_kernels.hip
+++ b/littoral-naval-warfare-marl_amd/csrc/lnw_kernels.hip
@@ -247,7 +247,7 @@
   }
   MaskBlocked mb{S.mask2, P.W16};
   bool sb = mb(sx, sy);
-  if (S.ctr) atomicAdd(&S.ctr[2], 1ull);
+  if (S.cold->ctr) atomicAdd(&S.cold->ctr[2], 1ull);
   return check_path_dev(mb, sb, P.G, type, sx, sy, tx, ty, open, ost);
 }
 
@@ -258,11 +258,11 @@
 
 __device__ inline uint32_t los_march_c(const KState &S, const uint32_t *mask, int W16, int x1,
                                        int y1, int x2, int y2) {
-  if (!S.ctr) return los_march<true>(mask, W16, x1, y1, x2, y2);
+  if (!S.cold->ctr) return los_march<true>(mask, W16, x1, y1, x2, y2);
   int n = 0;
   const uint32_t r = los_march<true>(mask, W16, x1, y1, x2, y2, &n);
-  atomicAdd(&S.ctr[0], 1ull);
-  atomicAdd(&S.ctr[1], (unsigned long long)n);
+  atomicAdd(&S.cold->ctr[0], 1ull);
+  atomicAdd(&S.cold->ctr[1], (unsigned long long)n);
   return r;
 }
 
@@ -358,8 +358,8 @@
     int k = COLB(c.bcnt, jj);
     if (k == 0) { COLB(c.border, acc.norder) = (uint8_t)jj; acc.norder++; }
     size_t slot = (size_t)(jj * S.nmax + k) * X.E + X.env;
-    S.bear_val[slot] = bearing;
-    S.bear_ship[slot] = (uint8_t)i;
+    S.cold->bear_val[slot] = bearing;
+    S.cold->bear_ship[slot] = (uint8_t)i;
     COLB(c.bcnt, jj) = (uint8_t)(k + 1);
   }
 }
@@ -385,8 +385,8 @@
     int k = COLB(c.bcnt, jj);
     if (k == 0) { COLB(c.border, acc.norder) = (uint8_t)jj; acc.norder++; }
     size_t slot = (size_t)(jj * S.nmax + k) * X.E + X.env;
-    S.bear_val[slot] = bearing;
-    S.bear_ship[slot] = (uint8_t)i;
+    S.cold->bear_val[slot] = bearing;
+    S.cold->bear_ship[slot] = (uint8_t)i;
     COLB(c.bcnt, jj) = (uint8_t)(k + 1);
   }
 }
@@ -442,8 +442,8 @@
   const int m = n - 1;
   FixAcc f;
   for (int k = 0; k < m; k++) {
-    uint8_t s1 = S.bear_ship[slot(k)], s2 = S.bear_ship[slot(k + 1)];
-    double b1 = S.bear_val[slot(k)], b2 = S.bear_val[slot(k + 1)];
+    uint8_t s1 = S.cold->bear_ship[slot(k)], s2 = S.cold->bear_ship[slot(k + 1)];
+    double b1 = S.cold->bear_val[slot(k)], b2 = S.cold->bear_val[slot(k + 1)];
     uint32_t p1 = COLW(c.pos_cur, s1), p2 = COLW(c.pos_cur, s2);
     double m1 = tan_fd(b1 * DEG2RAD);
     double m2 = tan_fd(b2 * DEG2RAD);
@@ -468,7 +468,7 @@
   for (int k = 0; k < BMAX; k++) {
     bv[k] = 0.0;
     bs[k] = 0;
-    if (k < n) { bv[k] = S.bear_val[slot(k)]; bs[k] = S.bear_ship[slot(k)]; }
+    if (k < n) { bv[k] = S.cold->bear_val[slot(k)]; bs[k] = S.cold->bear_ship[slot(k)]; }
   }
   double tv[BMAX], px[BMAX], py[BMAX];
 #pragma unroll
@@ -530,9 +530,9 @@
     if (!ok) { X.rng.err |= LNW_ERRF_ZERODIV; continue; }
     if (!isfinite(mx) || !isfinite(my)) { X.rng.err |= LNW_ERRF_NAN_ROUND; continue; }
     double rx = rint(mx), ry = rint(my);
-    if (S.ana.ew_log) {
+    if (S.cold->ana.ew_log) {
       const int fx = (int)fmin(fmax(rx, -32768.0), 32767.0), fy = (int)fmin(fmax(ry, -32768.0), 32767.0);
-      ana_record(S.ana.ew_log, S.ana.ew_count, S.ana.ew_cap, (uint32_t)(P.env_base + env),
+      ana_record(S.cold->ana.ew_log, S.cold->ana.ew_count, S.cold->ana.ew_cap, (uint32_t)(P.env_base + env),
                  (uint32_t)X.step | (uint32_t)(me >= P.nb) << 16, COLW(c.pos_cur, me),
                  (uint32_t)(uint16_t)fx | (uint32_t)(uint16_t)fy << 16);
     }
@@ -576,9 +576,9 @@
       const uint32_t pj = COLW(c.pos_cur, j);
       int n = 0;
       acc += los_march<false>(X.mask, P.W16, pos_x(pi), pos_y(pi), pos_x(pj), pos_y(pj), &n);
-      if (X.S.ctr) {
-        atomicAdd(&X.S.ctr[0], 1ull);
-        atomicAdd(&X.S.ctr[1], (unsigned long long)n);
+      if (X.S.cold->ctr) {
+        atomicAdd(&X.S.cold->ctr[0], 1ull);
+        atomicAdd(&X.S.cold->ctr[1], (unsigned long long)n);
       }
     }
   }
@@ -761,9 +761,9 @@
     const double mx = sumx / (double)(cnt - 1), my = sumy / (double)(cnt - 1);
     if (!isfinite(mx) || !isfinite(my)) { X.rng.err |= LNW_ERRF_NAN_ROUND; return; }
     const double rx = rint(mx), ry = rint(my);
-    if (S.ana.ew_log) {
+    if (S.cold->ana.ew_log) {
       const int fx = (int)fmin(fmax(rx, -32768.0), 32767.0), fy = (int)fmin(fmax(ry, -32768.0), 32767.0);
-      ana_record(S.ana.ew_log, S.ana.ew_count, S.ana.ew_cap, (uint32_t)(P.env_base + env),
+      ana_record(S.cold->ana.ew_log, S.cold->ana.ew_count, S.cold->ana.ew_cap, (uint32_t)(P.env_base + env),
                  (uint32_t)X.step | (uint32_t)(me >= P.nb) << 16, COLW(c.pos_cur, me),
                  (uint32_t)(uint16_t)fx | (uint32_t)(uint16_t)fy << 16);
     }
@@ -818,7 +818,7 @@
                                              __builtin_amdgcn_mbcnt_lo((uint32_t)bb, 0u)) << b;
       total += __popcll(bb) << b;
     }
-    if (S.ctr && rank == 0) atomicAdd(&S.ctr[3], (unsigned long long)total);
+    if (S.cold->ctr && rank == 0) atomicAdd(&S.cold->ctr[3], (unsigned long long)total);
     uint8_t *lor = (uint8_t *)c.observed;
     uint16_t *exr = (uint16_t *)(lor + WAVE);
     uint32_t *fixt = (uint32_t *)(lor + 3 * WAVE);
@@ -854,9 +854,9 @@
     auto draw = [&](int s, unsigned long long d) -> double {
       const int es = env - lane + s;
       if (tape) {
-        if (!S.tape_off) return 0.0;
-        const long long p = S.tape_off[es] + (long long)d;
-        return p < S.tape_off[es + 1] ? S.tape[p] : 0.0;
+        if (!S.cold->tape_off) return 0.0;
+        const long long p = S.cold->tape_off[es] + (long long)d;
+        return p < S.cold->tape_off[es + 1] ? S.cold->tape[p] : 0.0;
       }
       const unsigned long long gid = (unsigned long long)(P.env_base + es);
       return X.rng.gauss_philox(d, (uint32_t)gid, (uint32_t)(gid >> 32));
@@ -871,9 +871,9 @@
           w = 1u << 18;
         } else {
           const double rx = rint(mx), ry = rint(my);
-          if (S.ana.ew_log) {
+          if (S.cold->ana.ew_log) {
             const int fx = (int)fmin(fmax(rx, -32768.0), 32767.0), fy = (int)fmin(fmax(ry, -32768.0), 32767.0);
-            ana_record(S.ana.ew_log, S.ana.ew_count, S.ana.ew_cap, (uint32_t)(P.env_base + env - lane + s),
+            ana_record(S.cold->ana.ew_log, S.cold->ana.ew_count, S.cold->ana.ew_cap, (uint32_t)(P.env_base + env - lane + s),
                        (uint32_t)stp | (uint32_t)(me >= P.nb) << 16, c.pos_cur[me * PAD + s],
                        (uint32_t)(uint16_t)fx | (uint32_t)(uint16_t)fy << 16);
           }
@@ -933,7 +933,7 @@
         ZB = !fB && (ZA || zB);
       }
       int stA = 0, stB = 0;
-      if (S.ana.ew_log) {
+      if (S.cold->ana.ew_log) {
         stA = __shfl(X.step, sA);
         stB = __shfl(X.step, sB);
       }
@@ -1466,13 +1466,13 @@
     const KState &S = X.S;
     if (missile) {
       if (side == (P.side_blue ? 0 : 1)) {
-        ana_map(S.ana.heatmap, pa);
-        ana_map(S.ana.coldmap, pt);
-      }
-      if (S.ana.launch) ana_map(S.ana.launch + side * 10000, pa);
-    }
-    if (S.ana.eng_log)
-      ana_record(S.ana.eng_log, S.ana.eng_count, S.ana.eng_cap, (uint32_t)(P.env_base + X.env),
+        ana_map(S.cold->ana.heatmap, pa);
+        ana_map(S.cold->ana.coldmap, pt);
+      }
+      if (S.cold->ana.launch) ana_map(S.cold->ana.launch + side * 10000, pa);
+    }
+    if (S.cold->ana.eng_log)
+      ana_record(S.cold->ana.eng_log, S.cold->ana.eng_count, S.cold->ana.eng_cap, (uint32_t)(P.env_base + X.env),
                  (uint32_t)X.step | (uint32_t)side << 16 | (uint32_t)n << 24, pa, pt);
   }
   if (hit) {
@@ -1579,14 +1579,14 @@
   unsigned long long box_ctr = ((unsigned long long)(uint32_t)S.envi[7 * E + env]) << 32;
   for (int a = 0; a < P.A; a++) {
     size_t ai = (size_t)a * E + env;
-    int t = S.sp_types[a];
+    int t = S.cold->sp_types[a];
     int x, y;
-    if (S.sp_pos_env) {
-      x = S.sp_pos_env[((size_t)env * P.A + a) * 2];
-      y = S.sp_pos_env[((size_t)env * P.A + a) * 2 + 1];
+    if (S.cold->sp_pos_env) {
+      x = S.cold->sp_pos_env[((size_t)env * P.A + a) * 2];
+      y = S.cold->sp_pos_env[((size_t)env * P.A + a) * 2 + 1];
     } else {
-      x = S.sp_pos[2 * a];
-      y = S.sp_pos[2 * a + 1];
+      x = S.cold->sp_pos[2 * a];
+      y = S.cold->sp_pos[2 * a + 1];
     }
     if (box) {
       for (int tries = 0; tries < 64; tries++) {
@@ -1602,7 +1602,7 @@
         if (!(cell_bits(S.mask2, P.W16, bx, by) & 1u)) { x = bx; y = by; break; }
       }
     }
-    if (S.sp_randls[a]) {
+    if (S.cold->sp_randls[a]) {
       x = rng.randint(98, 99);
       y = rng.randint(48, 56);
     }
@@ -1639,12 +1639,14 @@
   r.g1 = (uint32_t)(gid >> 32);
   r.ctr = S.rng[env];
   r.err = 0;
-  r.tape = S.tape;
-  if (P.rng_mode == 1 && S.tape_off) {
-    r.tape_lo = S.tape_off[env];
-    r.tape_hi = S.tape_off[env + 1];
-  } else {
-    r.tape_lo = r.tape_hi = 0;
+  r.tape = nullptr;
+  r.tape_lo = r.tape_hi = 0;
+  if (P.rng_mode == 1) {
+    r.tape = S.cold->tape;
+    if (S.cold->tape_off) {
+      r.tape_lo = S.cold->tape_off[env];
+      r.tape_hi = S.cold->tape_off[env + 1];
+    }
   }
   return r;
 }
@@ -2556,7 +2558,7 @@
 template <int NB, int NR, bool CW, bool REFW, int UN, bool PS, bool SL>
 __device__ __forceinline__ void step_body(
     const KParams &P, KState S, void *actions, const uint8_t *row_kind, float *obs_b, float *obs_r,
-    float *rew_b, float *rew_r, int32_t *done_out, float *cog_out) {
+    float *rew_b, float *rew_r, int32_t *done_out, float *cog_out, unsigned long long t_entry = 0) {
   static_assert(UN == 1 || (NB > 0 && EPW == WAVE && !REFW), "units need the two-wave templated kernel");
   const int unit = UN > 1 ? (int)(threadIdx.x / (2 * WAVE)) : 0;
   const int lane = threadIdx.x & (WAVE - 1);
@@ -2606,6 +2608,9 @@
   }
   if (wid == 0) {
     prof_stamp(S, 0);
+#ifdef LNW_DIAG
+    prof_put(S, 13, t_entry);
+#endif
     prof_put(S, 30, (unsigned long long)__builtin_amdgcn_s_getreg((3 << 11) | 20));
     prof_put(S, 31, (unsigned long long)__builtin_amdgcn_s_getreg((31 << 11) | 4));
   } else if (wid == 1) {
@@ -3028,11 +3033,37 @@
   else write_obs(P, S, c, duct_col, obs_b, obs_r, env0, nenv, false);
 }
 
+__device__ __forceinline__ void kernarg_lines_prefetch() {
+#if defined(__HIP_DEVICE_COMPILE__)
+  const auto ka = __builtin_amdgcn_kernarg_segment_ptr();
+  uint32_t t0, t1, t2, t3, t4, t5, t6, t7, t8, t9, t10, t11, t12, t13;
+  asm volatile(
+      "s_load_dword %0, %14, 0x0\n\ts_load_dword %1, %14, 0x40\n\ts_load_dword %2, %14, 0x80\n\t"
+      "s_load_dword %3, %14, 0xc0\n\ts_load_dword %4, %14, 0x100\n\ts_load_dword %5, %14, 0x140\n\t"
+      "s_load_dword %6, %14, 0x180\n\ts_load_dword %7, %14, 0x1c0\n\ts_load_dword %8, %14, 0x200\n\t"
+      "s_load_dword %9, %14, 0x240\n\ts_load_dword %10, %14, 0x280\n\ts_load_dword %11, %14, 0x2c0\n\t"
+      "s_load_dword %12, %14, 0x300\n\ts_load_dword %13, %14, 0x340\n\t"
+      "s_waitcnt lgkmcnt(0)"
+      : "=&s"(t0), "=&s"(t1), "=&s"(t2), "=&s"(t3), "=&s"(t4), "=&s"(t5), "=&s"(t6), "=&s"(t7), "=&s"(t8),
+        "=&s"(t9), "=&s"(t10), "=&s"(t11), "=&s"(t12), "=&s"(t13)
+      : "s"(ka));
+  __builtin_amdgcn_sched_barrier(0);
+#endif
+}
+
 template <int NB, int NR, bool CW = false, bool REFW = false, int UN = 1, bool PS = false, bool SL = false>
 __global__ __launch_bounds__(NB > 0 && EPW == WAVE ? 2 * WAVE * UN : WAVE, NB > 0 ? 2 : 1) void step_kernel(
     KParams P, KState S, void *actions, const uint8_t *row_kind, float *obs_b, float *obs_r,
     float *rew_b, float *rew_r, int32_t *done_out, float *cog_out) {
+#ifdef LNW_DIAG
+  const unsigned long long t_entry = __builtin_amdgcn_s_memrealtime();
+  kernarg_lines_prefetch();
+  step_body<NB, NR, CW, REFW, UN, PS, SL>(P, S, actions, row_kind, obs_b, obs_r, rew_b, rew_r, done_out, cog_out,
+                                          t_entry);
+#else
+  kernarg_lines_prefetch();
   step_body<NB, NR, CW, REFW, UN, PS, SL>(P, S, actions, row_kind, obs_b, obs_r, rew_b, rew_r, done_out, cog_out);
+#endif
 }
 
 #include "lnw_group.inc"
@@ -3403,6 +3434,8 @@
   int device = 0;
   lnw_params params{};
   KParams kp{};
+  struct ColdSlot { KCold host; KCold *dev; };
+  std::vector<ColdSlot> cold_slots;
   int E = 0, nb = 0, nr = 0, A = 0, T = 0, nmax = 0;
   long long env_base = 0;
   int G = 0, W16 = 0;
@@ -3458,13 +3491,38 @@
   s.pos = h->pos; s.radar = h->radar; s.miss = h->miss; s.mkind = h->mkind; s.alive = h->alive;
   s.type = h->type; s.steps = h->steps; s.dist_lz = h->dist_lz; s.tl_cnt = h->tl_cnt; s.tl = h->tl;
   s.duct = h->duct; s.envi = h->envi; s.rng = h->rng; s.err = h->err;
-  s.bear_val = h->bear_val; s.bear_ship = h->bear_ship; s.atan_deg = h->d_atan;
-  s.grid = h->d_grid; s.gridf = h->d_gridf; s.winf = h->d_winf; s.dummy = h->d_dummy; s.prof = nullptr; s.ana = h->ana; s.ctr = h->ctr; s.mask2 = h->d_mask2; s.mvtab = h->d_mvtab; s.lostab = h->d_lostab;
-  s.tape = h->tape; s.tape_off = h->tape_off;
-  s.sp_types = h->sp_types; s.sp_pos = h->sp_pos; s.sp_randls = h->sp_randls;
-  s.sp_pos_env = h->sp_pos_env_on ? h->sp_pos_env : nullptr;
+  s.atan_deg = h->d_atan;
+  s.grid = h->d_grid; s.gridf = h->d_gridf; s.winf = h->d_winf; s.dummy = h->d_dummy; s.prof = nullptr; s.cold = nullptr; s.mask2 = h->d_mask2; s.mvtab = h->d_mvtab; s.lostab = h->d_lostab;
   s.nmax = h->nmax;
   return s;
+}
+
+int cold_commit(lnw_handle *h, ColdPtr *out) {
+  KCold c;
+  memset(&c, 0, sizeof c);
+  c.ana = h->ana;
+  c.tape = h->tape; c.tape_off = h->tape_off;
+  c.sp_types = h->sp_types; c.sp_pos = h->sp_pos; c.sp_randls = h->sp_randls;
+  c.sp_pos_env = h->sp_pos_env_on ? h->sp_pos_env : nullptr;
+  c.bear_val = h->bear_val; c.bear_ship = h->bear_ship;
+  c.ctr = h->ctr;
+  for (size_t i = h->cold_slots.size(); i-- > 0;)
+    if (memcmp(&h->cold_slots[i].host, &c, sizeof c) == 0) {
+      if (out) *out = (ColdPtr)h->cold_slots[i].dev;
+      return 0;
+    }
+  KCold *d = nullptr;
+  HIPCHK(hipSetDevice(h->device));
+  if (int rc = dalloc(h, &d, 1)) return rc;
+  HIPCHK(hipMemcpy(d, &c, sizeof c, hipMemcpyHostToDevice));
+  h->cold_slots.push_back({c, d});
+  if (out) *out = (ColdPtr)d;
+  return 0;
+}
+
+int launch_state(lnw_handle *h, KState &s) {
+  s = make_state(h);
+  return cold_commit(h, &s.cold);
 }
 
 size_t step_lds_bytes(const lnw_handle *h) {
@@ -3712,6 +3770,23 @@
                       "rows staged %.2f, stored %.2f us\n",
               nd, q0 / nd * us, q1 / nd * us, rb / nd * us, rc / nd * us);
   }
+#ifdef LNW_DIAG
+  {
+    double se = 0, sl = 0, me = 0;
+    int ne = 0;
+    for (int w = 0; w < nwg; w++) {
+      const unsigned long long *r = &t[(size_t)w * PROF_SLOTS];
+      if (!r[14] || !r[13] || r[13] > r[0]) continue;
+      ne++;
+      se += (double)(r[0] - r[13]);
+      sl += (double)(r[4] - r[0]);
+      if ((double)(r[0] - r[13]) > me) me = (double)(r[0] - r[13]);
+    }
+    if (ne)
+      fprintf(stderr, "[lnw prof] entry -> stamp 0 %.3f us (max %.2f), stamp 0 -> phase-L end %.3f us (%d quiet records)\n",
+              se / ne * us, me * us, sl / ne * us, ne);
+  }
+#endif
   if (nq)
     fprintf(stderr, "[lnw prof] quiet workgroups %d: M %.2f us, A*+barrier %.2f us, quiet test %.2f us, Q+barrier %.2f us; "
                     "tail: rewards %.2f, cog %.2f, env_tail+outputs %.2f us\n",
@@ -3735,11 +3810,11 @@
 
 int lnw_set_analytics(lnw_handle *h, const lnw_analytics *a) {
   if (!h) return fail(LNW_EINVAL, "null handle");
-  if (!a) { h->ana = lnw_analytics{}; return 0; }
+  if (!a) { h->ana = lnw_analytics{}; return cold_commit(h, nullptr); }
   if ((a->eng_log && (!a->eng_count || a->eng_cap < 0)) || (a->ew_log && (!a->ew_count || a->ew_cap < 0)))
     return fail(LNW_EINVAL, "analytics log without a counter or with a negative capacity");
   h->ana = *a;
-  return 0;
+  return cold_commit(h, nullptr);
 }
 
 int lnw_hit_tables(double *tab64, float *tab32) {
@@ -3978,7 +4053,7 @@
   h->tape = tape_dev;
   h->tape_off = (const long long *)tape_off_dev;
   HIPCHK(hipMemset(h->rng, 0, sizeof(unsigned long long) * h->E));
-  return 0;
+  return cold_commit(h, nullptr);
 }
 
 static int apply_side_types(lnw_handle *h, const int32_t *types, bool apply) {
@@ -4028,7 +4103,8 @@
     HIPCHK(hipMemcpyAsync(h->sp_pos_env, pos_dev, n * sizeof(int32_t), hipMemcpyDeviceToDevice, st));
   }
   h->sp_pos_env_on = pos_dev != nullptr;
-  KState s = make_state(h);
+  KState s;
+  if (int rc = launch_state(h, s)) return rc;
   reset_kernel<<<(h->E + 255) / 256, 256, 0, st>>>(h->kp, s, env_mask_dev);
   HIPCHK(hipGetLastError());
   return 0;
@@ -4053,7 +4129,8 @@
   k.no_obs = obs_blue_dev == nullptr ? 1 : 0;
   k.dbg_skip = h->dbg_skip;
   k.store_wt = h->store_wt;
-  KState s = make_state(h);
+  KState s;
+  if (int rc = launch_state(h, s)) return rc;
   k.qdirect = step_qdirect(h, k.epw) ? 1 : 0;
   size_t lds = step_launch_lds_bytes(h, k.epw);
   dim3 grid((h->E + k.epw - 1) / k.epw), block(WAVE);
@@ -4170,7 +4247,8 @@
       (red_env_stride && (red_env_stride < row_r || red_env_stride % 4)))
     return fail(LNW_EINVAL, "env stride: 0, or a multiple of 4 floats of at least the side's n * D");
   if (((uintptr_t)obs_blue_dev | (uintptr_t)obs_red_dev) & 15) return fail(LNW_EINVAL, "rows must be 16-B aligned");
-  KState s = make_state(h);
+  KState s;
+  if (int rc = launch_state(h, s)) return rc;
   size_t lds = step_lds_bytes(h);
   dim3 grid((h->E + h->kp.epw - 1) / h->kp.epw), block(WAVE);
   hipStream_t st = (hipStream_t)stream;
@@ -4341,13 +4419,13 @@
   if (hd.rng_mode == LNW_RNG_PHILOX) h->kp.seed = hd.seed;
   for (int i = 0; i < 2; i++) { h->kp.box_lo[i] = hd.box_lo[i]; h->kp.box_hi[i] = hd.box_hi[i]; }
   h->sp_pos_env_on = hd.pos_env_on != 0;
-  return 0;
+  return cold_commit(h, nullptr);
 }
 
 int lnw_set_counters(lnw_handle *h, uint64_t *counters_dev) {
   if (!h) return fail(LNW_EINVAL, "null handle");
   h->ctr = (unsigned long long *)counters_dev;
-  return 0;
+  return cold_commit(h, nullptr);
 }
 
 int lnw_set_reward_dtype(lnw_handle *h, int32_t f64) {
@@ -4406,7 +4484,8 @@
     return fail(LNW_EINVAL, "null argument");
   if (!h->terrain) return fail(LNW_ESTATE, "lnw_load_terrain must be called first");
   if (n <= 0) return 0;
-  KState s = make_state(h);
+  KState s;
+  if (int rc = launch_state(h, s)) return rc;
   move_batch_kernel<<<(unsigned)((n + WAVE - 1) / WAVE), WAVE, 0, (hipStream_t)stream>>>(
       h->kp, s, types_dev, pos_dev, act_dev, is_f32_dev, n, rounded_dev, ok_dev);
   HIPCHK(hipGetLastError());
@@ -4418,7 +4497,8 @@
   if (!h || !types_dev || !start_dev || !target_dev || !out_dev) return fail(LNW_EINVAL, "null argument");
   if (!h->terrain) return fail(LNW_ESTATE, "lnw_load_terrain must be called first");
   if (n <= 0) return 0;
-  KState s = make_state(h);
+  KState s;
+  if (int rc = launch_state(h, s)) return rc;
   path_query_kernel<<<(unsigned)((n + WAVE - 1) / WAVE), WAVE, 0, (hipStream_t)stream>>>(
       h->kp, s, types_dev, start_dev, target_dev, n, out_dev);
   HIPCHK(hipGetLastError());
@@ -4429,7 +4509,8 @@
   if (!h || !pairs_dev || !out_dev) return fail(LNW_EINVAL, "null argument");
   if (!h->terrain) return fail(LNW_ESTATE, "lnw_load_terrain must be called first");
   if (n <= 0) return 0;
-  KState s = make_state(h);
+  KState s;
+  if (int rc = launch_state(h, s)) return rc;
   los_query_kernel<<<(unsigned)((n + 255) / 256), 256, 0, (hipStream_t)stream>>>(h->kp, s, pairs_dev, n, out_dev);
   HIPCHK(hipGetLastError());
   return 0;
```

Result: faster. 1.664 billion env-steps/sec (median of 6 runs) (+2.5%).
